# lionl1106/Searchable-Generative-Image-Compression

Measured on AMD Instinct MI355X. Metric: images/sec end-to-end compress (enc+entropy+CLIP) at 256x256, higher is better.
Workload: dtype f32; 1 GPU; configs[1]: batch=32 256x256 encoder+entropy+CLIP compress per GPU, TiTok ViT-L hybrid encoder + ViT-B/32 CLIP, synthetic weights; global_batch=32

## Files before the change

### include/sgic.h

```cpp
#ifndef SGIC_H
#define SGIC_H
#include <stddef.h>
#include <stdint.h>

#ifdef __cplusplus
extern "C" {
#endif

typedef struct ihipStream_t *sgic_stream_t;

#define SGIC_OK 0
#define SGIC_EINVAL -1
#define SGIC_EHIP -2
#define SGIC_ENOSPC -3
#define SGIC_ENODEV -4

const char *sgic_last_error(void);
int sgic_version(void);
int sgic_device_count(void);


int sgic_pmf_to_quantized_cdf(const float *pmf, int n, int precision, uint32_t *cdf_out);

typedef struct sgic_cdf_table sgic_cdf_table;
int sgic_cdf_table_create(const int32_t *cdf, int rows, int cols, const int32_t *sizes, const int32_t *offsets,
                          sgic_cdf_table **out);
void sgic_cdf_table_destroy(sgic_cdf_table *t);

int sgic_rans_encode_batch(const sgic_cdf_table *t, const int16_t *d_sym, const int16_t *d_idx, int B,
                           int n_per_img, uint8_t *d_out, int cap, int32_t *d_off, int32_t *d_len,
                           int32_t *d_err, sgic_stream_t stream);

int sgic_rans_decode_init_batch(const uint8_t *d_streams, int cap, const int32_t *d_off, const int32_t *d_len,
                                int B, uint32_t *d_state, sgic_stream_t stream);
int sgic_rans_decode_batch(const sgic_cdf_table *t, const uint8_t *d_streams, int cap, const int32_t *d_off,
                           const int32_t *d_len, int B, uint32_t *d_state, const int16_t *d_idx, int n,
                           int idx_stride, int16_t *d_sym_out, int out_stride, sgic_stream_t stream);

size_t sgic_pack12_size(size_t n);
int sgic_pack12_batch(const int32_t *d_idx, int B, int n, uint8_t *d_out, sgic_stream_t stream);
int sgic_unpack12_batch(const uint8_t *d_in, int B, int n, int32_t *d_idx, sgic_stream_t stream);

int sgic_quant_step(const float *d_y, const float *d_scales, const float *d_means, int ld_sm, float *d_yhat,
                    int ld_yhat, int B, int H, int W, int C, int k, float thr, int16_t *d_sym, int16_t *d_idx,
                    sgic_stream_t stream);
int sgic_scale_to_index(const float *d_scales, long n, float thr, int16_t *d_idx, sgic_stream_t stream);
int sgic_index_step(const float *d_scales, int ld_sm, int B, int H, int W, int C, int k, float thr,
                    int16_t *d_idx, sgic_stream_t stream);
int sgic_index_margins(const float *d_scales, int ld_sm, int B, int H, int W, int C, int k, float thr, float *d_margin,
                       int16_t *d_alt, sgic_stream_t stream);
int sgic_dequant_step(const int16_t *d_sym, const float *d_means, int ld_sm, float *d_yhat, int ld_yhat, int B,
                      int H, int W, int C, int k, sgic_stream_t stream);

#define SGIC_ACT_NONE 0
#define SGIC_ACT_GELU 1
#define SGIC_ACT_SILU 2
#define SGIC_ACT_TANH 3
#define SGIC_ACT_LRELU 4

typedef struct sgic_profiler sgic_profiler;
typedef struct sgic_launch_opts {
  int tile_mode;
  int attn_mode;
  sgic_profiler *profiler;
  int w_packed;
  int a_packed;
} sgic_launch_opts;

int sgic_profiler_create(sgic_profiler **out);
void sgic_profiler_destroy(sgic_profiler *p);
int sgic_profiler_begin(sgic_profiler *p, int max_launches);
int sgic_profiler_end(sgic_profiler *p, float *ms_out, int cap, int *n_out);

int sgic_gemm_f32(const float *d_A, int lda, const float *d_W, int ldw, const float *d_bias, const float *d_R,
                  int ldr, float *d_C, int ldc, int M, int N, int K, int act, int a_seg, int a_seg_stride,
                  int c_seg, int c_seg_stride, const sgic_launch_opts *opts, sgic_stream_t stream);

int sgic_layernorm_f32(const float *d_x, int ldx, int xseg, int xseg_stride, const float *d_gamma,
                       const float *d_beta, float *d_y, int ldy, int yseg, int yseg_stride, int M, int C, float eps,
                       int act, sgic_stream_t stream);

int sgic_attention_f32(const float *d_q, int ldq, const float *d_k, int ldk, const float *d_v, int ldv,
                       float *d_out, int ldo, int L, int nseq, int nheads, const int32_t *d_rowmap,
                       const float *d_bias, const int32_t *d_biasvar, float scale, const sgic_launch_opts *opts,
                       sgic_stream_t stream);
int sgic_attention_window_f32(const float *d_q, int ldq, const float *d_k, int ldk, const float *d_v, int ldv,
                              float *d_out, int ldo, int L, int nseq, int nheads, const int32_t *d_rowmap,
                              const float *d_bias, const int32_t *d_biasvar, float scale, int q_tok0, int Lq,
                              const sgic_launch_opts *opts, sgic_stream_t stream);
int sgic_copy_blocks_f32(const float *d_src, long src_stride, float *d_dst, long dst_stride, long block_elems, int nblocks,
                         sgic_stream_t stream);

int sgic_im2col_patch(const float *d_x, int B, int C, int H, int W, int P, float mul, float add, int tile16,
                      float *d_out, sgic_stream_t stream);
int sgic_assemble_tokens(const float *d_emb, const float *d_cls, const float *d_pos, const float *d_lat,
                         const float *d_latpos, int N, int P, int T, int D, float *d_out, sgic_stream_t stream);
int sgic_add_rows_bcast(const float *d_in, int ldi, int iseg, const float *d_vec, float *d_out, int ldo, int oseg,
                        int Nn, int Lr, int D, sgic_stream_t stream);
int sgic_dwconv_nhwc(const float *d_x, const float *d_w, const float *d_bias, const float *d_prescale, float *d_y,
                     int B, int H, int W, int C, int k, int tile16, sgic_stream_t stream);
int sgic_im2col_2x2(const float *d_x, int B, int H, int W, int C, int tile16, float *d_out, sgic_stream_t stream);
int sgic_gated_lrelu(const float *d_x, float *d_out, int M, int C2, sgic_stream_t stream);
int sgic_colop(const float *d_x, int ldx, const float *d_v, int ldv, int vrows, float *d_y, int ldy, int M, int C,
               int mode, sgic_stream_t stream);
int sgic_fake2d_transpose(const float *d_in, long in_seq_stride, float *d_out, int N, int T, int D,
                          sgic_stream_t stream);
int sgic_vq_argmin(const float *d_z, int ldz, const float *d_codebook, int ncodes, int dim, int M, int l2norm,
                   int32_t *d_idx, sgic_stream_t stream);
int sgic_clip_preprocess(const float *d_x, long img_stride, long ch_stride, int ldx, int B, int H, int W, int OH,
                         int OW, int S, int top, int left, const int32_t *d_bounds_h, const int32_t *d_kk_h,
                         int ksize_h, const int32_t *d_bounds_v, const int32_t *d_kk_v, int ksize_v,
                         const float *mean3, const float *std3, uint8_t *d_tmp_u8, uint8_t *d_tmp_h, float *d_out,
                         sgic_stream_t stream);
int sgic_l2norm_u8(const float *d_x, int ldx, int M, int D, float *d_unit, uint8_t *d_q, sgic_stream_t stream);

int sgic_split3_f32(const float *d_x, int ld, int rows, int cols, int seg, int seg_stride, uint16_t *d_planes,
                    sgic_stream_t stream);
int sgic_split3_pack_f32(const float *d_x, int ld, int rows, int cols, uint16_t *d_planes, sgic_stream_t stream);
int sgic_gemm_split3_f32(const float *d_A, int lda, int a_seg, int a_seg_stride, uint16_t *d_Aplanes,
                         const uint16_t *d_Wplanes, const float *d_bias, const float *d_R, int ldr, float *d_C, int ldc,
                         uint16_t *d_Cplanes, int M, int N, int K, int act, int c_seg, int c_seg_stride,
                         const sgic_launch_opts *opts, sgic_stream_t stream);
int sgic_conv3x3_split3_f32(const uint16_t *d_in_planes, const uint16_t *d_Wplanes, const float *d_bias, const float *d_R,
                            int ldr, float *d_out, int ldc, int B, int H, int W, int Cin, int Cout, int act,
                            const sgic_launch_opts *opts, sgic_stream_t stream);
int sgic_groupnorm_nhwc_split3(const float *d_x, const float *d_gamma, const float *d_beta, int B, int H, int W, int C,
                               int groups, float eps, int swish, double *d_ws, float *d_stats, uint16_t *d_halo_planes,
                               sgic_stream_t stream);
int sgic_halo_copy_split3(const float *d_in, int B, int H, int W, int C, int upsample2x, int tile16, uint16_t *d_halo_planes,
                          sgic_stream_t stream);
int sgic_attention_split3_f32(const float *d_q, int ldq, const float *d_k, int ldk, const float *d_v, int ldv,
                              uint16_t *d_out_planes, long rows, int L, int nseq, int nheads, const int32_t *d_rowmap,
                              const float *d_bias, const int32_t *d_biasvar, float scale, const sgic_launch_opts *opts,
                              sgic_stream_t stream);
int sgic_attention_window_split3_f32(const float *d_q, int ldq, const float *d_k, int ldk, const float *d_v, int ldv,
                                     uint16_t *d_out_planes, long rows, int L, int nseq, int nheads, const int32_t *d_rowmap,
                                     const float *d_bias, const int32_t *d_biasvar, float scale, int q_tok0, int Lq,
                                     const sgic_launch_opts *opts, sgic_stream_t stream);
int sgic_layernorm_split3_f32(const float *d_x, int ldx, int xseg, int xseg_stride, const float *d_gamma,
                              const float *d_beta, uint16_t *d_planes, int M, int C, float eps, int act,
                              sgic_stream_t stream);

int sgic_gemm_batched_f32(const float *d_A, int lda, long strideA, const float *d_W, int ldw, long strideW,
                          const float *d_bias, const float *d_R, int ldr, long strideR, float *d_C, int ldc,
                          long strideC, int M, int N, int K, int act, int batch, const sgic_launch_opts *opts,
                          sgic_stream_t stream);
int sgic_conv3x3_f32(const float *d_in_halo, const float *d_W, const float *d_bias, const float *d_R, int ldr,
                     float *d_out, int ldc, int B, int H, int W, int Cin, int Cout, int act, const sgic_launch_opts *opts,
                     sgic_stream_t stream);
int sgic_groupnorm_nhwc(const float *d_x, const float *d_gamma, const float *d_beta, int B, int H, int W, int C,
                        int groups, float eps, int swish, int halo_out, double *d_ws, float *d_stats, float *d_y,
                        sgic_stream_t stream);
int sgic_halo_copy(const float *d_in, int B, int H, int W, int C, int upsample2x, int tile16, float *d_out,
                   sgic_stream_t stream);
int sgic_softmax_rows(const float *d_x, float *d_y, long M, int L, float scale, sgic_stream_t stream);
int sgic_pixel_shuffle2_tm16(const float *d_in, int B, int H, int W, int C, float *d_out, sgic_stream_t stream);
int sgic_assemble_dec_tokens(const float *d_emb, const float *d_cls, const float *d_mask, const float *d_pos,
                             const float *d_latpos, int N, int P, int T, int D, float *d_out, sgic_stream_t stream);
int sgic_codebook_gather_norm(const int32_t *d_idx, const float *d_codebook, int M, int dim, int ld, float *d_out,
                              sgic_stream_t stream);
int sgic_nhwc3_to_nchw_clamp(const float *d_in, int ld, int B, int H, int W, float *d_out, sgic_stream_t stream);

int sgic_topk_rows(float *d_scores, int nq, int n, int k, float *d_out_scores, int32_t *d_out_idx, sgic_stream_t stream);

int sgic_search_codes_u8_work_bytes(int nq, int n, int D, int k, int splits, int *splits_used, size_t *bytes);
int sgic_search_codes_u8(const uint8_t *d_q, const float *d_rq, const uint8_t *d_db, const float *d_rdb, int nq, int n, int D, int k,
                         int splits, uint8_t *d_work, size_t work_bytes, float *d_out_scores, int32_t *d_out_idx,
                         sgic_stream_t stream);

int sgic_search_codes_f32q_work_bytes(int nq, int n, int D, int k, int splits, int *splits_used, size_t *bytes);
int sgic_search_codes_f32q(const float *d_q, const uint8_t *d_db, const float *d_rdb, int nq, int n, int D, int k, int splits,
                           uint8_t *d_work, size_t work_bytes, float *d_out_scores, int32_t *d_out_idx, sgic_stream_t stream);

int sgic_search_range_u8(const uint8_t *d_q, const float *d_rq, const uint8_t *d_db, const float *d_rdb, int nq, int n, int D,
                         float threshold, int self_join, int splits, long long capacity, uint64_t *d_count, int32_t *d_out_q,
                         int32_t *d_out_d, float *d_out_score, sgic_stream_t stream);

int sgic_search_range_f32q(const float *d_q, const uint8_t *d_db, const float *d_rdb, int nq, int n, int D, float threshold,
                           int splits, long long capacity, uint64_t *d_count, int32_t *d_out_q, int32_t *d_out_d,
                           float *d_out_score, sgic_stream_t stream);

int sgic_pad_replicate(const float *d_in, float *d_out, int BC, int H, int W, int pl, int pr, int pt, int pb,
                       sgic_stream_t stream);

int sgic_u8hwc_to_f32chw_pad(const uint8_t *d_in, float *d_out, int B, int H, int W, int pl, int pr, int pt, int pb,
                             sgic_stream_t stream);

int sgic_u8canvas_to_f32chw_pad(const uint8_t *d_in, const int32_t *h_hw, float *d_out, int B, int Hc, int Wc, int OH, int OW,
                                sgic_stream_t stream);
int sgic_clip_resize_coeffs(int in_size, int out_size, int ksize, int32_t *d_bounds, int32_t *d_kk, sgic_stream_t stream);
int sgic_clip_preprocess_ragged_workspace(int B, const int32_t *h_geo, int S, size_t *bytes);
int sgic_clip_preprocess_ragged(const float *d_x, long img_stride, long ch_stride, int ldx, int B, const int32_t *h_geo, int S,
                                const float *mean3, const float *std3, uint8_t *d_work, size_t work_bytes, float *d_out,
                                sgic_stream_t stream);
int sgic_clip_preprocess_u8canvas_workspace(int B, const int32_t *h_geo, int S, size_t *bytes);
int sgic_clip_preprocess_u8canvas(const uint8_t *d_canvas, int Hc, int Wc, int B, const int32_t *h_geo, int S, const float *mean3,
                                  const float *std3, uint8_t *d_work, size_t work_bytes, float *d_out, sgic_stream_t stream);

int sgic_jpeg_decode_batch(const int32_t *d_params, const uint8_t *d_scan, const uint8_t *d_tabs, const int32_t *d_segs,
                           const uint16_t *d_quant, int32_t *d_work_params, uint16_t *d_work_quant, int16_t *d_coef,
                           uint8_t *d_planes, uint8_t *d_out, int32_t *d_err, int B, int H, int W, int max_blocks,
                           sgic_stream_t stream);

int sgic_jpeg_decode_scans_batch(const int32_t *d_params, const int32_t *d_descs, const uint8_t *d_scan, const uint8_t *d_tabs,
                                 const int32_t *d_segs, const uint16_t *d_quant, int32_t *d_work_params, uint16_t *d_work_quant,
                                 int16_t *d_coef, uint8_t *d_planes, uint8_t *d_out, int32_t *d_err, int B, int H, int W,
                                 long total_blocks, int max_blocks, const int32_t *h_level_start, int nlevels,
                                 sgic_stream_t stream);

int sgic_embed_tokens(const int32_t *d_ids, const float *d_table, const float *d_pos, float *d_out, int B, int L, int D,
                      int vocab, sgic_stream_t stream);
int sgic_gather_eot_rows(const int32_t *d_ids, const float *d_x, int ldx, float *d_out, int B, int L, int D,
                         sgic_stream_t stream);

#ifdef __cplusplus
}
#endif
#endif
```

### searchable-generative-image-compression_amd/clip.py

```python
import math

import numpy as np
import torch

from . import ops
from ._lib import call
from .config import ClipConfig
from .encoder import RabW, rab_forward, rab_forward_last

_PREC = 22


def _bicubic(x):
    a = -0.5
    x = abs(x)
    if x < 1.0:
        return ((a + 2.0) * x - (a + 3.0)) * x * x + 1
    if x < 2.0:
        return (((x - 5) * x + 8) * x - 4) * a
    return 0.0


def pil_coeffs(in_size, out_size):
    scale = in_size / out_size
    fscale = max(scale, 1.0)
    support = 2.0 * fscale
    ksize = int(math.ceil(support)) * 2 + 1
    bounds = np.zeros((out_size, 2), dtype=np.int32)
    kk = np.zeros((out_size, ksize), dtype=np.int32)
    ss = 1.0 / fscale
    for xx in range(out_size):
        center = (xx + 0.5) * scale
        xmin = int(center - support + 0.5)
        xmin = max(xmin, 0)
        xmax = int(center + support + 0.5)
        xmax = min(xmax, in_size) - xmin
        w = [_bicubic((x + xmin - center + 0.5) * ss) for x in range(xmax)]
        ww = 0.0
        for v in w:
            ww += v
        if ww != 0.0:
            w = [v / ww for v in w]
        for x, v in enumerate(w):
            kk[xx, x] = int(-0.5 + v * (1 << _PREC)) if v < 0 else int(0.5 + v * (1 << _PREC))
        bounds[xx] = (xmin, xmax)
    return bounds, kk, ksize


def resize_geometry(H, W, S):
    if H <= W:
        OH, OW = S, int(S * W / H)
    else:
        OH, OW = int(S * H / W), S
    top = int(round((OH - S) / 2.0))
    left = int(round((OW - S) / 2.0))
    return OH, OW, top, left


class ClipHIP:
    def __init__(self, sd, cfg: ClipConfig, device, p="clip.visual", prune_last=True):
        self.cfg, self.device = cfg, device
        self.prune_last = prune_last
        g = lambda k: sd[f"{p}.{k}"].to(device=device, dtype=torch.float32).contiguous()
        Wd = cfg.width
        self.conv_w = sd[f"{p}.conv1.weight"].reshape(Wd, -1).to(device).contiguous()
        self.cls = g("class_embedding").reshape(1, Wd).contiguous()
        self.pos = g("positional_embedding")
        self.lnpre_w, self.lnpre_b = g("ln_pre.weight"), g("ln_pre.bias")
        self.blocks = [RabW(sd, f"{p}.transformer.resblocks.{i}", device) for i in range(cfg.layers)]
        self.lnpost_w, self.lnpost_b = g("ln_post.weight"), g("ln_post.bias")
        self.projT = sd[f"{p}.proj"].t().to(device).contiguous()
        self.mean = np.asarray(cfg.mean, dtype=np.float32)
        self.std = np.asarray(cfg.std, dtype=np.float32)
        self._coef = {}

    def _coeffs(self, H, W):
        key = (H, W)
        if key not in self._coef:
            S = self.cfg.image_size
            OH, OW, top, left = resize_geometry(H, W, S)
            bh, kh, ksh = pil_coeffs(W, OW)
            bv, kv, ksv = pil_coeffs(H, OH)
            d = lambda a: torch.from_numpy(np.ascontiguousarray(a)).to(self.device)
            self._coef[key] = (OH, OW, top, left, d(bh), d(kh), ksh, d(bv), d(kv), ksv)
        return self._coef[key]

    def preprocess(self, x, H=None, W=None, hw=None):
        if hw is not None:
            return self._preprocess_ragged(x, hw)
        B, _, Hp, Wp = x.shape
        H, W = H or Hp, W or Wp
        S = self.cfg.image_size
        OH, OW, top, left, bh, kh, ksh, bv, kv, ksv = self._coeffs(H, W)
        u8 = torch.empty(B * 3 * H * W, dtype=torch.uint8, device=x.device)
        th = torch.empty(B * 3 * H * OW, dtype=torch.uint8, device=x.device)
        out = torch.empty(B, 3, S, S, dtype=torch.float32, device=x.device)
        import ctypes
        call("sgic_clip_preprocess", ops._p(x), ctypes.c_long(x.stride(0)), ctypes.c_long(x.stride(1)), int(x.stride(2)),
             B, H, W, OH, OW, S, top, left, ops._p(bh), ops._p(kh), ksh, ops._p(bv), ops._p(kv), ksv,
             self.mean.ctypes.data_as(ctypes.c_void_p), self.std.ctypes.data_as(ctypes.c_void_p), ops._p(u8), ops._p(th),
             ops._p(out))
        return out

    def _preprocess_ragged(self, x, hw):
        import ctypes
        B, _, Hp, Wp = x.shape
        hw = np.asarray(hw, dtype=np.int64).reshape(B, 2)
        if (hw <= 0).any() or (hw[:, 0] > Hp).any() or (hw[:, 1] > Wp).any():
            raise ValueError(f"extents {hw.tolist()} outside the {Hp}x{Wp} batch")
        S = self.cfg.image_size
        geo = np.array([(h, w) + resize_geometry(h, w, S) for h, w in hw.tolist()], dtype=np.int32)
        nbytes = ctypes.c_size_t(0)
        call("sgic_clip_preprocess_ragged_workspace", B, geo, S, ctypes.byref(nbytes))
        work = torch.empty(nbytes.value, dtype=torch.uint8, device=x.device)
        out = torch.empty(B, 3, S, S, dtype=torch.float32, device=x.device)
        call("sgic_clip_preprocess_ragged", ops._p(x), ctypes.c_long(x.stride(0)), ctypes.c_long(x.stride(1)), int(x.stride(2)), B, geo, S,
             self.mean, self.std, ops._p(work), ctypes.c_size_t(nbytes.value), ops._p(out))
        return out

    def preprocess_u8(self, canvas, hw):
        if canvas.dim() != 4 or canvas.shape[3] != 3 or canvas.dtype != torch.uint8:
            raise ValueError(f"canvas must be (B, Hc, Wc, 3) uint8, got {tuple(canvas.shape)} {canvas.dtype}")
        B, Hc, Wc, _ = canvas.shape
        hw = np.asarray(hw, dtype=np.int64).reshape(B, 2)
        if (hw <= 0).any() or (hw[:, 0] > Hc).any() or (hw[:, 1] > Wc).any():
            raise ValueError(f"extents {hw.tolist()} outside the {Hc}x{Wc} canvas")
        S = self.cfg.image_size
        geo = np.array([(h, w) + resize_geometry(h, w, S) for h, w in hw.tolist()], dtype=np.int32)
        return ops.clip_preprocess_u8canvas(canvas.contiguous(), geo, S, self.mean, self.std)

    def tower(self, pre):
        cfg = self.cfg
        B = pre.shape[0]
        g = cfg.image_size // cfg.patch
        L = g * g + 1
        A = ops.im2col_patch(pre, cfg.patch, 1.0, 0.0, tile16=False)
        emb = ops.gemm(A, self.conv_w)
        X = ops.assemble_tokens(emb, self.cls, self.pos, None, None, B, g * g, 0, cfg.width)
        ops.layernorm(X, self.lnpre_w, self.lnpre_b, out=X)
        if self.prune_last and L > 32:
            for w in self.blocks[:-1]:
                rab_forward(X, w, L, B, cfg.heads)
            pooled = rab_forward_last(X, self.blocks[-1], L, B, cfg.heads, 0, 32, keep=1)
            ops.layernorm(pooled, self.lnpost_w, self.lnpost_b, out=pooled)
        else:
            for w in self.blocks:
                rab_forward(X, w, L, B, cfg.heads)
            pooled = ops.layernorm(X, self.lnpost_w, self.lnpost_b, M=B, x_seg=(1, L))
        z = ops.gemm(pooled, self.projT)
        return ops.l2norm_u8(z)

    def encode(self, x, H=None, W=None, hw=None):
        return self.tower(self.preprocess(x, H, W, hw))

    def encode_u8(self, canvas, hw):
        return self.tower(self.preprocess_u8(canvas, hw))


class ClipTextHIP:

    def __init__(self, sd, cfg: ClipConfig, device, p="clip"):
        self.cfg, self.device = cfg, device
        g = lambda k: sd[f"{p}.{k}"].to(device=device, dtype=torch.float32).contiguous()
        self.table, self.pos = g("token_embedding.weight"), g("positional_embedding")
        self.blocks = [RabW(sd, f"{p}.transformer.resblocks.{i}", device) for i in range(cfg.t_layers)]
        self.lnf_w, self.lnf_b = g("ln_final.weight"), g("ln_final.bias")
        self.projT = sd[f"{p}.text_projection"].t().to(device=device, dtype=torch.float32).contiguous()
        L = self.L = (cfg.ctx + 3) & ~3
        if L != cfg.ctx:
            self.pos = torch.cat([self.pos, torch.zeros(L - cfg.ctx, cfg.t_width, device=device)]).contiguous()
        self.causal = torch.full((L, L), float("-inf")).triu_(1).reshape(1, L, L).to(device).contiguous()

    def encode_text(self, tokens):
        cfg = self.cfg
        ids = torch.as_tensor(np.asarray(tokens.cpu() if torch.is_tensor(tokens) else tokens)).to(torch.int32)
        if ids.dim() != 2 or ids.shape[1] != cfg.ctx:
            raise ValueError(f"tokens must be (B, {cfg.ctx}), got {tuple(ids.shape)}")
        if self.L != cfg.ctx:
            ids = torch.nn.functional.pad(ids, (0, self.L - cfg.ctx))
        ids = ids.to(self.device).contiguous()
        B, L, D = ids.shape[0], self.L, cfg.t_width
        X = torch.empty(B * L, D, dtype=torch.float32, device=self.device)
        call("sgic_embed_tokens", ops._p(ids), ops._p(self.table), ops._p(self.pos), ops._p(X), B, L, D, cfg.vocab)
        for w in self.blocks:
            rab_forward(X, w, L, B, cfg.t_heads, bias=self.causal)
        pooled = torch.empty(B, D, dtype=torch.float32, device=self.device)
        call("sgic_gather_eot_rows", ops._p(ids), ops._p(X), D, ops._p(pooled), B, L, D)
        ops.layernorm(pooled, self.lnf_w, self.lnf_b, out=pooled)
        z = ops.gemm(pooled, self.projT)
        return ops.l2norm_u8(z)[0]
```

### searchable-generative-image-compression_amd/csrc/gemm_split.hip

```cpp
#include <type_traits>

#include "common.h"
#include "gemm_act.h"
#include "profiler.h"
#include "split3.h"

typedef float f32x16 __attribute__((ext_vector_type(16)));
typedef float f32x4 __attribute__((ext_vector_type(4)));
typedef __bf16 bf16x8 __attribute__((ext_vector_type(8)));
typedef unsigned u32x4 __attribute__((ext_vector_type(4)));

template <bool PACK>
__global__ __launch_bounds__(256) void split3_rows_kernel(const float *__restrict__ x, int ld, int rows, int cols, int seg,
                                                          int seg_stride, unsigned short *__restrict__ planes) {
  const int c8 = cols >> 3;
  const long total = (long)rows * c8, plane = (long)rows * cols;
  for (long i = (long)blockIdx.x * 256 + threadIdx.x; i < total; i += (long)gridDim.x * 256) {
    const int r = (int)(i / c8), c = (int)(i - (long)r * c8) * 8;
    const size_t src = (seg ? (size_t)(r / seg) * seg_stride + (r % seg) : (size_t)r) * ld + c;
    const f32x4 v0 = *reinterpret_cast<const f32x4 *>(x + src), v1 = *reinterpret_cast<const f32x4 *>(x + src + 4);
    unsigned p1[4], p2[4], p3[4];
    s3_split_pair(v0[0], v0[1], p1[0], p2[0], p3[0]);
    s3_split_pair(v0[2], v0[3], p1[1], p2[1], p3[1]);
    s3_split_pair(v1[0], v1[1], p1[2], p2[2], p3[2]);
    s3_split_pair(v1[2], v1[3], p1[3], p2[3], p3[3]);
    const size_t dst = PACK ? ((size_t)(c >> 5) * rows + r) * 32 + (c & 31) : (size_t)r * cols + c;
    *reinterpret_cast<u32x4 *>(planes + dst) = u32x4{p1[0], p1[1], p1[2], p1[3]};
    *reinterpret_cast<u32x4 *>(planes + plane + dst) = u32x4{p2[0], p2[1], p2[2], p2[3]};
    *reinterpret_cast<u32x4 *>(planes + 2 * plane + dst) = u32x4{p3[0], p3[1], p3[2], p3[3]};
  }
}

template <int N, int I = 0, typename F>
__device__ __forceinline__ void s3_for(F &&f) {
  if constexpr (I < N) {
    f(IntC<I>{});
    s3_for<N, I + 1>(f);
  }
}

struct S3Args {
  const unsigned short *A, *W;
  const float *bias, *R;
  float *C;
  int M, N, K, ldr, ldc, act;
  int c_seg, c_seg_stride;
  long a_plane, w_plane;
  unsigned short *Cp;
  long c_plane;
  int vec_epilogue;
  int conv_C, conv_H, conv_W;
  int m_base;
  int w_packed;
  int a_packed, a_rows;
  int c_rows;
};

template <int BM, int BN, int PASSES>
__device__ __forceinline__ void s3_tile_epilogue(const S3Args &g, f32x4 (&acc)[BM][BN], float *ep, int em0, int en0, int wm, int wn, int lane) {
  const int l16 = lane & 15, lq = lane >> 4;
  if (g.vec_epilogue) {
    constexpr int BMP = BM / PASSES, RM = 16 * BMP, CN = 16 * BN, LDW = CN + 4, LPR = CN / 4, RPI = 64 / LPR, NIT = (RM + RPI - 1) / RPI;
    constexpr bool EXACT = (64 % LPR) == 0 && (RM % RPI) == 0;
    static_assert(BM % PASSES == 0, "epilogue passes");
    const int c4 = (lane % LPR) * 4, r0 = lane / LPR;
    const bool lane_on = EXACT || lane < RPI * LPR;
    const int n = en0 + wn + c4;
    const bool colok = n < g.N && lane_on;
    const int nc = colok ? n : 0;
    f32x4 bv = {0.f, 0.f, 0.f, 0.f};
    if (g.bias && colok) bv = *reinterpret_cast<const f32x4 *>(g.bias + n);
    s3_for<PASSES>([&](auto pass_c) __attribute__((always_inline)) {
      constexpr int pass = decltype(pass_c)::value;
#pragma unroll
      for (int i = 0; i < BMP; i++)
#pragma unroll
        for (int j = 0; j < BN; j++) *reinterpret_cast<f32x4 *>(ep + (i * 16 + l16) * LDW + j * 16 + 4 * lq) = acc[pass * BMP + i][j];
      asm volatile("s_waitcnt lgkmcnt(0)" ::: "memory");
      const int wmp = wm + pass * RM;
      auto run = [&](auto act_c, auto res_c, auto pl_c) __attribute__((always_inline)) {
        constexpr int ACT = decltype(act_c)::value;
        constexpr bool HASR = decltype(res_c)::value != 0, PLANES = decltype(pl_c)::value != 0;
        constexpr int EB = NIT < 8 ? NIT : 8;
#pragma unroll
        for (int b = 0; b < NIT; b += EB) {
          f32x4 cv[EB], rv[EB];
#pragma unroll
          for (int q = 0; q < EB; ++q) {
            const int rr = EXACT ? (b + q) * RPI + r0 : min((b + q) * RPI + r0, RM - 1);
            cv[q] = *reinterpret_cast<const f32x4 *>(ep + rr * LDW + c4);
            if constexpr (HASR) rv[q] = *reinterpret_cast<const f32x4 *>(g.R + (size_t)(min(em0 + wmp + rr, g.M - 1) + g.m_base) * g.ldr + nc);
          }
#pragma unroll
          for (int q = 0; q < EB; ++q) {
            if (!EXACT && (b + q >= NIT || (b + q) * RPI + r0 >= RM)) continue;
            const int m = em0 + wmp + (b + q) * RPI + r0;
            f32x4 v = cv[q];
#pragma unroll
            for (int t = 0; t < 4; t++) v[t] = apply_act_c<ACT>(v[t] + bv[t]);
            if constexpr (HASR) v += rv[q];
            if (colok && m < g.M) {
              if constexpr (PLANES) {
                s3_store4(g.Cp, g.c_plane, s3_pack_off(m + g.m_base, n, g.c_rows), v);
              } else {
                const int mm = m + g.m_base;
                const size_t crow = g.c_seg ? (size_t)(mm / g.c_seg) * g.c_seg_stride + (mm % g.c_seg) : (size_t)mm;
                *reinterpret_cast<f32x4 *>(g.C + crow * g.ldc + n) = v;
              }
            }
          }
        }
      };
      auto run_act = [&](auto act_c) __attribute__((always_inline)) {
        if (g.Cp) {
          if (g.R) run(act_c, IntC<1>{}, IntC<1>{});
          else run(act_c, IntC<0>{}, IntC<1>{});
        } else {
          if (g.R) run(act_c, IntC<1>{}, IntC<0>{});
          else run(act_c, IntC<0>{}, IntC<0>{});
        }
      };
      switch (g.act) {
        case ACT_GELU: run_act(IntC<ACT_GELU>{}); break;
        case ACT_SILU: run_act(IntC<ACT_SILU>{}); break;
        case ACT_TANH: run_act(IntC<ACT_TANH>{}); break;
        case ACT_LRELU: run_act(IntC<ACT_LRELU>{}); break;
        default: run_act(IntC<ACT_NONE>{}); break;
      }
    });
    return;
  }
  auto run = [&](auto act_c, auto res_c) __attribute__((always_inline)) {
    constexpr int ACT = decltype(act_c)::value;
    constexpr bool HASR = decltype(res_c)::value != 0;
#pragma unroll
    for (int j = 0; j < BN; j++) {
      const int n = en0 + wn + j * 16 + 4 * lq;
#pragma unroll
      for (int i = 0; i < BM; i++) {
        const int m = em0 + wm + i * 16 + l16;
        if (m >= g.M) continue;
        const int mm = m + g.m_base;
        const size_t crow = g.c_seg ? (size_t)(mm / g.c_seg) * g.c_seg_stride + (mm % g.c_seg) : (size_t)mm;
#pragma unroll
        for (int t = 0; t < 4; t++) {
          if (n + t < g.N) {
            float o = apply_act_c<ACT>(acc[i][j][t] + (g.bias ? g.bias[n + t] : 0.f));
            if constexpr (HASR) o += g.R[(size_t)mm * g.ldr + n + t];
            g.C[crow * g.ldc + n + t] = o;
          }
        }
      }
    }
  };
  auto run_act = [&](auto act_c) __attribute__((always_inline)) {
    if (g.R) run(act_c, IntC<1>{});
    else run(act_c, IntC<0>{});
  };
  switch (g.act) {
    case ACT_GELU: run_act(IntC<ACT_GELU>{}); break;
    case ACT_SILU: run_act(IntC<ACT_SILU>{}); break;
    case ACT_TANH: run_act(IntC<ACT_TANH>{}); break;
    case ACT_LRELU: run_act(IntC<ACT_LRELU>{}); break;
    default: run_act(IntC<ACT_NONE>{}); break;
  }
}

#ifndef S3_ABLATE
#define S3_ABLATE 0
#endif
#ifndef S3_DMA_VARIANT
#define S3_DMA_VARIANT 0
#endif
#ifdef S3_STAMPS
__device__ unsigned long long s3_stamps[4] = {~0ull, 0ull, 0ull, 0ull};
__device__ unsigned long long s3_wg[1024][6];
#endif

template <int WAVES_M, int WAVES_N, int BM, int BN, int NS, int KS, bool PERSIST>
__global__ __launch_bounds__(64 * WAVES_M * WAVES_N, (2 * 3 * 16 * (BM * WAVES_M + BN * WAVES_N) * 64 * KS <= 80 * 1024 && WAVES_M * WAVES_N == 8) ? 2 : 1)
void gemm_split3_kernel(S3Args g) {
#ifdef S3_STAMPS
  const unsigned long long st_rt0 = __builtin_amdgcn_s_memrealtime(), st_c0 = __builtin_amdgcn_s_memtime();
#endif
  static_assert(KS == 1 || KS == 2, "32-k slices per stage");
  static_assert(!PERSIST || NS == 1, "the persistent walk is built on the one-register-set pipeline");
  constexpr int NT = 64 * WAVES_M * WAVES_N, TM = 16 * BM * WAVES_M, TN = 16 * BN * WAVES_N;
  constexpr int ROWB = 64 * KS, SL = 4 * KS;
  constexpr int CA = (TM * SL + NT - 1) / NT, CW = (TN * SL + NT - 1) / NT;
  constexpr int APLANE = TM * ROWB, WPLANE = TN * ROWB, STAGE = 3 * (APLANE + WPLANE);
  constexpr int HB = BN >= 2 ? BN / 2 : BN;
  static_assert((NT / SL) % 16 == 0, "a thread's staged rows must share their swizzle term");
  extern __shared__ __attribute__((aligned(16))) unsigned char smem[];

  const int tiles_m = (g.M + TM - 1) / TM, tiles_n = (g.N + TN - 1) / TN, nwg = tiles_m * tiles_n;
  int m0, n0;
  auto locate = [&](int t) __attribute__((always_inline)) {
    const int q = nwg >> 3, r = nwg & 7, xcd = t & 7, within = t >> 3;
    t = (xcd < r ? xcd * (q + 1) : r * (q + 1) + (xcd - r) * q) + within;
    const int per_group = 8 * tiles_n, group = t / per_group, first_m = group * 8, gsz = min(tiles_m - first_m, 8),
              in_group = t - group * per_group;
    m0 = (first_m + in_group % gsz) * TM;
    n0 = (in_group / gsz) * TN;
  };
  int tile = blockIdx.x;
  locate(tile);
  const int tid = threadIdx.x, lane = tid & 63, wave = tid >> 6;
  const int wm = (wave / WAVES_N) * (16 * BM), wn = (wave % WAVES_N) * (16 * BN);
  auto swz = [](int row) __attribute__((always_inline)) {
    if constexpr (KS == 1) {
      const int gq = (row >> 2) & 3;
      return (((gq ^ (gq >> 1)) & 1) << 1) | (gq >> 1);
    } else {
      return (row >> 1) & 7;
    }
  };
  const int srow = tid / SL, sslot = tid % SL;
  const int sw = srow * ROWB + ((sslot ^ swz(srow)) * 16);
  const unsigned short *aptr[CA], *wptr[CW];
  auto setup = [&]() __attribute__((always_inline)) {
#pragma unroll
    for (int i = 0; i < CA; i++) {
      const int am = min(m0 + srow + i * (NT / SL), g.M - 1);
      if (g.conv_C) {
        const int hw = g.conv_H * g.conv_W, b = am / hw, r = am - b * hw, y = r / g.conv_W, x = r - y * g.conv_W;
        const size_t pix = ((size_t)b * (g.conv_H + 2) + y) * (g.conv_W + 2) + x;
        aptr[i] = g.a_packed ? g.A + ((size_t)(sslot >> 2) * g.a_rows + pix) * 32 + (sslot & 3) * 8 : g.A + pix * g.conv_C + sslot * 8;
      } else if (g.a_packed) {
        aptr[i] = g.A + ((size_t)(sslot >> 2) * g.a_rows + am) * 32 + (sslot & 3) * 8;
      } else {
        aptr[i] = g.A + (size_t)am * g.K + sslot * 8;
      }
    }
#pragma unroll
    for (int i = 0; i < CW; i++) {
      const size_t wr = (size_t)min(n0 + srow + i * (NT / SL), g.N - 1);
      wptr[i] = g.w_packed ? g.W + ((size_t)(sslot >> 2) * g.N + wr) * 32 + (sslot & 3) * 8 : g.W + wr * g.K + sslot * 8;
    }
  };
  setup();
  const bool a_on = CA * NT == TM * SL || srow < TM, w_on = CW * NT == TN * SL || srow < TN;
  u32x4 ra[NS][3][CA], rw[NS][3][CW];
  auto issue = [&](int k0, auto set_c) __attribute__((always_inline)) {
    constexpr int S = decltype(set_c)::value;
    if ((S3_ABLATE & 1) && k0 > 0) return;
    size_t ka = g.a_packed ? (size_t)k0 * g.a_rows : (size_t)k0;
    if (g.conv_C) {
      const int tap = k0 / g.conv_C, c0 = k0 - tap * g.conv_C, ky = tap / 3, kx = tap - 3 * ky;
      ka = g.a_packed ? ((size_t)(c0 >> 5) * g.a_rows + ky * (g.conv_W + 2) + kx) * 32 : (size_t)((ky * (g.conv_W + 2) + kx) * g.conv_C + c0);
    }
    const size_t kw = g.w_packed ? (size_t)k0 * g.N : (size_t)k0;
#pragma unroll
    for (int p = 0; p < 3; p++) {
#pragma unroll
      for (int i = 0; i < CA; i++) ra[S][p][i] = *reinterpret_cast<const u32x4 *>(aptr[i] + p * g.a_plane + ka);
#pragma unroll
      for (int i = 0; i < CW; i++) rw[S][p][i] = *reinterpret_cast<const u32x4 *>(wptr[i] + p * g.w_plane + kw);
    }
  };
  auto store = [&](int buf, auto set_c) __attribute__((always_inline)) {
    constexpr int S = decltype(set_c)::value;
    if ((S3_ABLATE & 2) && buf > 0) return;
    unsigned char *base = smem + buf * STAGE + sw;
#pragma unroll
    for (int p = 0; p < 3; p++) {
      if (a_on) {
#pragma unroll
        for (int i = 0; i < CA; i++) *reinterpret_cast<u32x4 *>(base + p * APLANE + i * (NT / SL) * ROWB) = ra[S][p][i];
      }
      if (w_on) {
#pragma unroll
        for (int i = 0; i < CW; i++) *reinterpret_cast<u32x4 *>(base + 3 * APLANE + p * WPLANE + i * (NT / SL) * ROWB) = rw[S][p][i];
      }
    }
  };
  f32x4 acc[BM][BN];
  const int l16 = lane & 15, lq = lane >> 4;
  int foff[KS];
#pragma unroll
  for (int ks = 0; ks < KS; ks++) foff[ks] = l16 * ROWB + (((4 * ks + lq) ^ swz(l16)) * 16);
  const int abase = wm * ROWB, bbase = 3 * APLANE + wn * ROWB;
  bf16x8 wf[3][BN], af[2][3];
  bool frag_reads = true;
  auto read_w = [&](int buf, int j, int ks) __attribute__((always_inline)) {
    if ((S3_ABLATE & 8) && !frag_reads) return;
    const unsigned char *base = smem + buf * STAGE + bbase + j * 16 * ROWB + foff[ks];
#pragma unroll
    for (int p = 0; p < 3; p++) wf[p][j] = *reinterpret_cast<const bf16x8 *>(base + p * WPLANE);
  };
  auto read_a = [&](int buf, int i, int set, int ks) __attribute__((always_inline)) {
    if ((S3_ABLATE & 8) && !frag_reads) return;
    const unsigned char *base = smem + buf * STAGE + abase + i * 16 * ROWB + foff[ks];
#pragma unroll
    for (int p = 0; p < 3; p++) af[set][p] = *reinterpret_cast<const bf16x8 *>(base + p * APLANE);
  };
  auto block = [&](int i, int j, int set) __attribute__((always_inline)) {
    f32x4 c = acc[i][j];
    c = __builtin_amdgcn_mfma_f32_16x16x32_bf16(wf[0][j], af[set][2], c, 0, 0, 0);
    c = __builtin_amdgcn_mfma_f32_16x16x32_bf16(wf[2][j], af[set][0], c, 0, 0, 0);
    c = __builtin_amdgcn_mfma_f32_16x16x32_bf16(wf[1][j], af[set][1], c, 0, 0, 0);
    c = __builtin_amdgcn_mfma_f32_16x16x32_bf16(wf[0][j], af[set][1], c, 0, 0, 0);
    c = __builtin_amdgcn_mfma_f32_16x16x32_bf16(wf[1][j], af[set][0], c, 0, 0, 0);
    c = __builtin_amdgcn_mfma_f32_16x16x32_bf16(wf[0][j], af[set][0], c, 0, 0, 0);
    acc[i][j] = c;
  };
  constexpr int BKS = 32 * KS;
  const int nk = g.K / BKS;
  auto tile_prologue = [&]() __attribute__((always_inline)) {
#pragma unroll
    for (int i = 0; i < BM; i++)
#pragma unroll
      for (int j = 0; j < BN; j++) acc[i][j] = f32x4{0.f, 0.f, 0.f, 0.f};
    store(0, IntC<0>{});
    if constexpr (NS == 1) {
      if (nk > 1) issue(BKS, IntC<0>{});
    } else {
      s3_for<NS>([&](auto u_c) __attribute__((always_inline)) {
        constexpr int J = decltype(u_c)::value + 1;
        if (J < nk) issue(J * BKS, IntC<J % NS>{});
      });
    }
    asm volatile("s_waitcnt lgkmcnt(0)" ::: "memory");
    __builtin_amdgcn_s_barrier();
#pragma unroll
    for (int j = BN - HB; j < BN; j++) read_w(0, j, 0);
    read_a(0, 0, 0, 0);
    if (S3_ABLATE & 8) {
#pragma unroll
      for (int j = 0; j < BN; j++) read_w(0, j, 0);
      read_a(0, 0, 1, 0);
      frag_reads = false;
    }
  };
  issue(0, IntC<0>{});
  auto compute = [&](int cur, auto ks_c, bool more) __attribute__((always_inline)) {
    constexpr int KSI = decltype(ks_c)::value;
    constexpr bool LAST = KSI == KS - 1;
    const int nxt = cur ^ 1;
    if constexpr (BN >= 2) {
#pragma unroll
      for (int j = 0; j < BN - HB; j++) read_w(cur, j, KSI);
    }
#pragma unroll
    for (int i = 0; i < BM; i++) {
      const int set = i & 1;
      if (i + 1 < BM) read_a(cur, i + 1, set ^ 1, KSI);
#pragma unroll
      for (int j = BN - HB; j < BN; j++) block(i, j, set);
      if (i == BM - 1) {
        if constexpr (LAST) {
          if constexpr (NS == 1) {
            constexpr int NMF1 = 6 * (BM * BN - (BN - HB)), NDW = 3 * (CA + CW), NDR1 = 3 * (BN - HB) + 3 * (BM - 1);
#pragma unroll
            for (int q = 0; q < NMF1; q++) {
              __builtin_amdgcn_sched_group_barrier(0x008, 1, 0);
              if (q < NDW) __builtin_amdgcn_sched_group_barrier(0x200, 1, 0);
              else if (q < 2 * NDW) __builtin_amdgcn_sched_group_barrier(0x020, 1, 0);
              if (q % 4 == 0 && q / 4 < NDR1) __builtin_amdgcn_sched_group_barrier(0x100, 1, 0);
            }
          }
          asm volatile("s_waitcnt lgkmcnt(0)" ::: "memory");
          if (!(S3_ABLATE & 4)) __builtin_amdgcn_s_barrier();
          if (more) {
#pragma unroll
            for (int j = BN - HB; j < BN; j++) read_w(nxt, j, 0);
            read_a(nxt, 0, BM == 1 ? 0 : (BM & 1), 0);
          }
        } else {
#pragma unroll
          for (int j = BN - HB; j < BN; j++) read_w(cur, j, KSI + 1);
          read_a(cur, 0, BM == 1 ? 0 : (BM & 1), KSI + 1);
        }
      }
      if constexpr (BN >= 2) {
#pragma unroll
        for (int j = 0; j < BN - HB; j++) block(i, j, set);
      }
    }
  };
  static_assert((BM == 1 && BN == 1) || (BM % 2) == 0, "A row 0 of the next slice must land in set 0, free at that point");
  auto tile_mainloop = [&]() __attribute__((always_inline)) {
    auto stage_mfma = [&](int cur, bool more) __attribute__((always_inline)) {
      s3_for<KS>([&](auto ks_c) __attribute__((always_inline)) { compute(cur, ks_c, more); });
    };
    if constexpr (NS == 1) {
      auto stage = [&](int kt, auto store_c, auto issue_c) __attribute__((always_inline)) {
        constexpr bool ST = decltype(store_c)::value, IS = decltype(issue_c)::value;
        if constexpr (ST) store((kt & 1) ^ 1, IntC<0>{});
        if constexpr (IS) issue((kt + 2) * BKS, IntC<0>{});
        stage_mfma(kt & 1, ST);
      };
      using T = std::true_type;
      using F = std::false_type;
      int kt = 0;
      for (; kt + 2 < nk; ++kt) stage(kt, T{}, T{});
      if (kt + 1 < nk) {
        stage(kt, T{}, F{});
        ++kt;
      }
      stage(kt, F{}, F{});
    } else {
      for (int base = 0; base < nk; base += NS) {
        s3_for<NS>([&](auto u_c) __attribute__((always_inline)) {
          constexpr int U = decltype(u_c)::value;
          const int kt = base + U;
          if (kt < nk) {
            const bool more = kt + 1 < nk;
            if (more) {
              store((kt & 1) ^ 1, IntC<(U + 1) % NS>{});
              if (kt + 1 + NS < nk) issue((kt + 1 + NS) * BKS, IntC<(U + 1) % NS>{});
            }
            stage_mfma(kt & 1, more);
          }
        });
      }
    }
  };

  auto tile_epilogue = [&](int em0, int en0) __attribute__((always_inline)) {
    s3_tile_epilogue<BM, BN, 1>(g, acc, reinterpret_cast<float *>(smem) + wave * (16 * BM * (16 * BN + 4)), em0, en0, wm, wn, lane);
  };

#ifdef S3_STAMPS
  unsigned long long ph_pro = 0, ph_main = 0, ph_epi = 0, ph_tiles = 0;
#endif
  for (;;) {
#ifdef S3_STAMPS
    const unsigned long long ph0 = __builtin_amdgcn_s_memtime();
#endif
    tile_prologue();
#ifdef S3_STAMPS
    const unsigned long long ph1 = __builtin_amdgcn_s_memtime();
// ... 262 lines not shown
    if (!more_tiles) break;
  }
}

template <int WAVES_M, int WAVES_N, int BM, int BN, int KS, int RING>
__global__ __launch_bounds__(64 * WAVES_M * WAVES_N, 1)
void gemm_split3_ring_kernel(S3Args g) {
  constexpr int NW = WAVES_M * WAVES_N, TM = 16 * BM * WAVES_M, TN = 16 * BN * WAVES_N;
  constexpr int ROWB = 64, PA = TM / 16, PW = TN / 16, PP = PA + PW, NP = 3 * PP * KS;
  constexpr int C = (NP + NW - 1) / NW;
  constexpr int APLANE = TM * ROWB, WPLANE = TN * ROWB, SLICE = 3 * (APLANE + WPLANE), STEP = KS * SLICE;
  static_assert(RING >= 3 && (RING - 2) * C <= 63, "vmcnt is a 6-bit counter");
  static_assert(NW * 16 * BM * (16 * BN + 4) * 4 <= RING * STEP, "the epilogue's per-wave slices fit the ring");
  extern __shared__ __attribute__((aligned(16))) unsigned char smem[];

  const int tiles_m = (g.M + TM - 1) / TM, tiles_n = (g.N + TN - 1) / TN, nwg = tiles_m * tiles_n;
  int m0, n0;
  {
    int t = blockIdx.x;
    const int q = nwg >> 3, r = nwg & 7, xcd = t & 7, within = t >> 3;
    t = (xcd < r ? xcd * (q + 1) : r * (q + 1) + (xcd - r) * q) + within;
    const int per_group = 8 * tiles_n, group = t / per_group, first_m = group * 8, gsz = min(tiles_m - first_m, 8),
              in_group = t - group * per_group;
    m0 = (first_m + in_group % gsz) * TM;
    n0 = (in_group / gsz) * TN;
  }
  const int tid = threadIdx.x, lane = tid & 63, wave = __builtin_amdgcn_readfirstlane(tid >> 6);
  const int wm = (wave / WAVES_N) * (16 * BM), wn = (wave % WAVES_N) * (16 * BN);
  auto swz = [](int row) __attribute__((always_inline)) {
    const int gq = (row >> 2) & 3;
    return (((gq ^ (gq >> 1)) & 1) << 1) | (gq >> 1);
  };
  const int prow = lane >> 2, pslot = (lane & 3) ^ swz(prow);
  const char *src[C];
  size_t kmul[C];
  unsigned dst[C];
#pragma unroll
  for (int i = 0; i < C; i++) {
    const int f = (wave + NW * i) % NP, ks = f / (3 * PP), rem = f - ks * (3 * PP), p = rem / PP, r = rem - p * PP;
    const bool isA = r < PA;
    const int rw = isA ? min(m0 + r * 16 + prow, g.M - 1) : min(n0 + (r - PA) * 16 + prow, g.N - 1);
    const unsigned short *base = isA ? g.A + p * g.a_plane : g.W + p * g.w_plane;
    const bool packed = isA ? g.a_packed != 0 : g.w_packed != 0;
    const size_t prows = isA ? (size_t)g.a_rows : (size_t)g.N;
    src[i] = reinterpret_cast<const char *>(base + (packed ? ((size_t)ks * prows + rw) * 32 : (size_t)rw * g.K + ks * 32)) + pslot * 16;
    kmul[i] = packed ? prows * (64 * KS) : (size_t)(64 * KS);
    dst[i] = (unsigned)(ks * SLICE + (isA ? p * APLANE + r * 1024 : 3 * APLANE + p * WPLANE + (r - PA) * 1024));
  }
  auto dma = [&](int step, int slot) __attribute__((always_inline)) {
    unsigned char *sbase = smem + slot * STEP;
#pragma unroll
    for (int i = 0; i < C; i++)
      __builtin_amdgcn_global_load_lds((s3_glb_void *)(src[i] + (size_t)step * kmul[i]), (s3_lds_void *)(sbase + dst[i]), 16, 0, 0);
  };
  f32x4 acc[BM][BN];
#pragma unroll
  for (int i = 0; i < BM; i++)
#pragma unroll
    for (int j = 0; j < BN; j++) acc[i][j] = f32x4{0.f, 0.f, 0.f, 0.f};
  const int l16 = lane & 15, lq = lane >> 4;
  const int foff = l16 * ROWB + ((lq ^ swz(l16)) * 16);
  const int abase = wm * ROWB + foff, bbase = 3 * APLANE + wn * ROWB + foff;
  bf16x8 af[2][KS][BM][3], wf[2][KS][BN][3];
  auto read_frags = [&](int slot, auto set_c) __attribute__((always_inline)) {
    constexpr int S = decltype(set_c)::value;
    const unsigned char *sbase = smem + slot * STEP;
#pragma unroll
    for (int ks = 0; ks < KS; ks++) {
#pragma unroll
      for (int p = 0; p < 3; p++) {
#pragma unroll
        for (int i = 0; i < BM; i++) af[S][ks][i][p] = *reinterpret_cast<const bf16x8 *>(sbase + ks * SLICE + p * APLANE + i * 16 * ROWB + abase);
#pragma unroll
        for (int j = 0; j < BN; j++) wf[S][ks][j][p] = *reinterpret_cast<const bf16x8 *>(sbase + ks * SLICE + p * WPLANE + j * 16 * ROWB + bbase);
      }
    }
  };
  auto compute = [&](auto set_c) __attribute__((always_inline)) {
    constexpr int S = decltype(set_c)::value;
    constexpr int TW[6] = {0, 2, 1, 0, 1, 0}, TA[6] = {2, 0, 1, 1, 0, 0};
#pragma unroll
    for (int ks = 0; ks < KS; ks++)
#pragma unroll
      for (int t = 0; t < 6; t++)
#pragma unroll
        for (int i = 0; i < BM; i++)
#pragma unroll
          for (int j = 0; j < BN; j++)
            acc[i][j] = __builtin_amdgcn_mfma_f32_16x16x32_bf16(wf[S][ks][j][TW[t]], af[S][ks][i][TA[t]], acc[i][j], 0, 0, 0);
  };
  const int nsteps = g.K / (32 * KS);
  {
    const int npro = min(RING - 1, nsteps);
    for (int s = 0; s < npro; s++) dma(s, s);
    if (npro == RING - 1) asm volatile("s_waitcnt vmcnt(%0)" ::"n"((RING - 2) * C) : "memory");
    else asm volatile("s_waitcnt vmcnt(0)" ::: "memory");
    __builtin_amdgcn_s_barrier();
    read_frags(0, IntC<0>{});
  }
  int slot_next = 1 % RING;
  int slot_fill = (RING - 1) % RING;
  auto iter = [&](int s, auto set_c) __attribute__((always_inline)) {
    constexpr int S = decltype(set_c)::value;
    if (s + 1 < nsteps) {
      if (s + RING - 2 <= nsteps - 1) asm volatile("s_waitcnt vmcnt(%0) lgkmcnt(0)" ::"n"((RING - 3) * C) : "memory");
      else asm volatile("s_waitcnt vmcnt(0) lgkmcnt(0)" ::: "memory");
      __builtin_amdgcn_s_barrier();
      if (s + RING - 1 < nsteps) dma(s + RING - 1, slot_fill);
      read_frags(slot_next, IntC<S ^ 1>{});
      slot_next = slot_next + 1 == RING ? 0 : slot_next + 1;
      slot_fill = slot_fill + 1 == RING ? 0 : slot_fill + 1;
    }
    compute(set_c);
  };
  for (int s = 0; s < nsteps; s += 2) {
    iter(s, IntC<0>{});
    if (s + 1 < nsteps) iter(s + 1, IntC<1>{});
  }
  asm volatile("s_waitcnt vmcnt(0) lgkmcnt(0)" ::: "memory");
  __builtin_amdgcn_s_barrier();
  s3_tile_epilogue<BM, BN, 1>(g, acc, reinterpret_cast<float *>(smem) + wave * (16 * BM * (16 * BN + 4)), m0, n0, wm, wn, lane);
}

extern "C" int sgic_split3_f32(const float *d_x, int ld, int rows, int cols, int seg, int seg_stride, uint16_t *d_planes,
                               sgic_stream_t stream) {
  SGIC_REQUIRE(d_x && d_planes && rows > 0 && cols > 0, "null/empty");
  SGIC_REQUIRE((cols & 7) == 0 && (ld & 3) == 0 && ld >= cols, "cols % 8, ld % 4");
  SGIC_REQUIRE(((uintptr_t)d_x & 15) == 0 && ((uintptr_t)d_planes & 15) == 0, "16-byte alignment");
  SGIC_REQUIRE(seg >= 0 && (seg == 0 || seg_stride >= seg), "row segment map");
  const long total = (long)rows * (cols >> 3);
  const unsigned grid = (unsigned)min((total + 255) / 256, 256L * 16);
  split3_rows_kernel<false><<<grid, 256, 0, to_stream(stream)>>>(d_x, ld, rows, cols, seg, seg_stride, d_planes);
  return sgic::check_launch("split3_rows_kernel");
}

extern "C" int sgic_split3_pack_f32(const float *d_x, int ld, int rows, int cols, uint16_t *d_planes, sgic_stream_t stream) {
  SGIC_REQUIRE(d_x && d_planes && rows > 0 && cols > 0, "null/empty");
  SGIC_REQUIRE((cols & 31) == 0 && (ld & 3) == 0 && ld >= cols, "cols % 32, ld % 4");
  SGIC_REQUIRE(((uintptr_t)d_x & 15) == 0 && ((uintptr_t)d_planes & 15) == 0, "16-byte alignment");
  const long total = (long)rows * (cols >> 3);
  const unsigned grid = (unsigned)min((total + 255) / 256, 256L * 16);
  split3_rows_kernel<true><<<grid, 256, 0, to_stream(stream)>>>(d_x, ld, rows, cols, 0, 0, d_planes);
  return sgic::check_launch("split3_rows_kernel<pack>");
}

#define SGIC_SPLIT3_TILE_MODES 31

template <int WAVES_M, int WAVES_N, int BM, int BN, int NS, int KS = 1, bool PERSIST = false>
static int s3_launch(const S3Args &g, hipStream_t st, hipEvent_t ev_start, hipEvent_t ev_stop) {
  constexpr int NT = 64 * WAVES_M * WAVES_N, TM = 16 * BM * WAVES_M, TN = 16 * BN * WAVES_N;
  constexpr int LDS = 2 * 3 * (TM + TN) * 64 * KS;
  static bool attr_set[64] = {};
  auto kernel = gemm_split3_kernel<WAVES_M, WAVES_N, BM, BN, NS, KS, PERSIST>;
  int dev = 0;
  SGIC_HIP(hipGetDevice(&dev));
  if (dev < 0 || dev >= 64 || !attr_set[dev]) {
    SGIC_HIP(hipFuncSetAttribute(reinterpret_cast<const void *>(kernel), hipFuncAttributeMaxDynamicSharedMemorySize, LDS));
    if (dev >= 0 && dev < 64) attr_set[dev] = true;
  }
  unsigned ntiles = (unsigned)(((g.M + TM - 1) / TM) * ((g.N + TN - 1) / TN));
  const dim3 grid(PERSIST ? (ntiles < 256u ? ntiles : 256u) : ntiles);
  if (ev_start || ev_stop) {
    hipExtLaunchKernelGGL(kernel, grid, dim3(NT), LDS, st, ev_start, ev_stop, 0, g);
  } else {
    kernel<<<grid, NT, LDS, st>>>(g);
  }
  return sgic::check_launch("gemm_split3_kernel");
}

template <int WAVES_M, int WAVES_N, int BM, int BN, bool PERSIST = false, bool WS1 = false>
static int s3_launch_dma(const S3Args &g, hipStream_t st, hipEvent_t ev_start, hipEvent_t ev_stop) {
  constexpr int NT = 64 * WAVES_M * WAVES_N, TM = 16 * BM * WAVES_M, TN = 16 * BN * WAVES_N;
  constexpr int LDS = WS1 ? 3 * (2 * TM + TN) * 64 : 2 * 3 * (TM + TN) * 64;
  static_assert(LDS <= 160 * 1024, "LDS of a CU");
  static bool attr_set[64] = {};
  auto kernel = gemm_split3_dma_kernel<WAVES_M, WAVES_N, BM, BN, PERSIST, WS1>;
  int dev = 0;
  SGIC_HIP(hipGetDevice(&dev));
  if (dev < 0 || dev >= 64 || !attr_set[dev]) {
    SGIC_HIP(hipFuncSetAttribute(reinterpret_cast<const void *>(kernel), hipFuncAttributeMaxDynamicSharedMemorySize, LDS));
    if (dev >= 0 && dev < 64) attr_set[dev] = true;
  }
  unsigned ntiles = (unsigned)(((g.M + TM - 1) / TM) * ((g.N + TN - 1) / TN));
  const dim3 grid(PERSIST ? (ntiles < 256u ? ntiles : 256u) : ntiles);
  if (ev_start || ev_stop) {
    hipExtLaunchKernelGGL(kernel, grid, dim3(NT), LDS, st, ev_start, ev_stop, 0, g);
  } else {
    kernel<<<grid, NT, LDS, st>>>(g);
  }
  return sgic::check_launch("gemm_split3_dma_kernel");
}

template <int WAVES_M, int WAVES_N, int BM, int BN, int KS, int RING>
static int s3_launch_ring(const S3Args &g, hipStream_t st, hipEvent_t ev_start, hipEvent_t ev_stop) {
  constexpr int NT = 64 * WAVES_M * WAVES_N, TM = 16 * BM * WAVES_M, TN = 16 * BN * WAVES_N;
  constexpr int LDS = RING * KS * 3 * (TM + TN) * 64;
  static_assert(LDS <= 160 * 1024, "LDS of a CU");
  static bool attr_set[64] = {};
  auto kernel = gemm_split3_ring_kernel<WAVES_M, WAVES_N, BM, BN, KS, RING>;
  int dev = 0;
  SGIC_HIP(hipGetDevice(&dev));
  if (dev < 0 || dev >= 64 || !attr_set[dev]) {
    SGIC_HIP(hipFuncSetAttribute(reinterpret_cast<const void *>(kernel), hipFuncAttributeMaxDynamicSharedMemorySize, LDS));
    if (dev >= 0 && dev < 64) attr_set[dev] = true;
  }
  const dim3 grid((unsigned)(((g.M + TM - 1) / TM) * ((g.N + TN - 1) / TN)));
  if (ev_start || ev_stop) {
    hipExtLaunchKernelGGL(kernel, grid, dim3(NT), LDS, st, ev_start, ev_stop, 0, g);
  } else {
    kernel<<<grid, NT, LDS, st>>>(g);
  }
  return sgic::check_launch("gemm_split3_ring_kernel");
}

static int s3_mode(const S3Args &g, int mode, hipStream_t st, hipEvent_t e0, hipEvent_t e1) {
  const bool dma_ok = (size_t)(g.a_packed ? 32 : g.K) * 2 * 256 < (1ull << 31) && (size_t)(g.w_packed ? 32 : g.K) * 2 * 256 < (1ull << 31) &&
                      (!g.conv_C || (size_t)(g.conv_W + 2) * (g.a_packed ? 32 : g.conv_C) * 2 * 1024 < (1ull << 31));
  switch (mode) {
    case 1: return dma_ok ? s3_launch_dma<2, 4, 4, 4>(g, st, e0, e1) : s3_launch<2, 4, 2, 2, 1>(g, st, e0, e1);
    case 10: return dma_ok ? s3_launch_dma<2, 4, 4, 4, true>(g, st, e0, e1) : s3_launch<2, 4, 2, 2, 1>(g, st, e0, e1);
#ifndef S3_MICRO_BIG_ONLY
    case 14: return dma_ok ? s3_launch_dma<4, 2, 4, 4>(g, st, e0, e1) : s3_launch<2, 4, 2, 2, 1>(g, st, e0, e1);
    case 15: return dma_ok ? s3_launch_dma<4, 2, 4, 4, true>(g, st, e0, e1) : s3_launch<2, 4, 2, 2, 1>(g, st, e0, e1);
    case 28: return dma_ok ? s3_launch_dma<2, 4, 4, 3>(g, st, e0, e1) : s3_launch<2, 4, 4, 2, 1>(g, st, e0, e1);
    case 29: return dma_ok ? s3_launch_dma<2, 4, 4, 3, true>(g, st, e0, e1) : s3_launch<2, 4, 4, 2, 1>(g, st, e0, e1);
    case 30: return dma_ok ? s3_launch_dma<2, 4, 8, 4, false, true>(g, st, e0, e1) : s3_launch<2, 4, 2, 2, 1>(g, st, e0, e1);
    case 16: return dma_ok ? s3_launch_dma<2, 4, 4, 2>(g, st, e0, e1) : s3_launch<2, 4, 4, 2, 1>(g, st, e0, e1);
    case 17: return dma_ok ? s3_launch_dma<2, 4, 4, 2, true>(g, st, e0, e1) : s3_launch<2, 4, 4, 2, 1, 1, true>(g, st, e0, e1);
    case 2: return s3_launch<2, 4, 4, 2, 1>(g, st, e0, e1);
    case 18: return (!g.conv_C && g.K % 64 == 0) ? s3_launch_ring<2, 2, 1, 1, 2, 6>(g, st, e0, e1) : s3_mode(g, 4, st, e0, e1);
    case 19: return (!g.conv_C && g.K % 64 == 0) ? s3_launch_ring<2, 2, 2, 1, 2, 4>(g, st, e0, e1) : s3_mode(g, 4, st, e0, e1);
    case 20: return (!g.conv_C && g.K % 64 == 0) ? s3_launch_ring<2, 2, 1, 2, 2, 4>(g, st, e0, e1) : s3_mode(g, 4, st, e0, e1);
    case 21: return !g.conv_C ? s3_launch_ring<2, 2, 2, 2, 1, 6>(g, st, e0, e1) : s3_mode(g, 3, st, e0, e1);
    case 22: return !g.conv_C ? s3_launch_ring<2, 4, 2, 1, 1, 6>(g, st, e0, e1) : s3_mode(g, 3, st, e0, e1);
    case 23: return !g.conv_C ? s3_launch_ring<1, 4, 5, 1, 1, 5>(g, st, e0, e1) : s3_mode(g, 3, st, e0, e1);
    case 24: return !g.conv_C ? s3_launch_ring<1, 3, 5, 1, 1, 6>(g, st, e0, e1) : s3_mode(g, 3, st, e0, e1);
    case 25: return (!g.conv_C && g.K % 64 == 0) ? s3_launch_ring<2, 3, 1, 1, 2, 5>(g, st, e0, e1) : s3_mode(g, 4, st, e0, e1);
    case 11: return s3_launch<2, 4, 4, 2, 1, 1, true>(g, st, e0, e1);
    case 3: return s3_launch<2, 2, 2, 2, 4>(g, st, e0, e1);
    case 4: return (g.K % 64 == 0 && g.conv_C % 64 == 0) ? s3_launch<2, 2, 1, 1, 3, 2>(g, st, e0, e1) : s3_launch<2, 2, 1, 1, 6>(g, st, e0, e1);
    default: return s3_launch<2, 4, 2, 2, 1>(g, st, e0, e1);
#else
    default: return SGIC_EINVAL;
#endif
  }
}

static int s3_dispatch(const S3Args &g, const sgic_launch_opts *opts, hipStream_t st) {
  const int M = g.M, N = g.N, K = g.K;
  int mode = opts ? opts->tile_mode : 0;
  SGIC_REQUIRE(mode >= 0 && mode <= SGIC_SPLIT3_TILE_MODES, "tile_mode");
  if (!mode) {
    const long t256 = (long)((M + 127) / 128) * ((N + 255) / 256), t128 = (long)((M + 127) / 128) * ((N + 127) / 128),
               t64 = (long)((M + 63) / 64) * ((N + 63) / 64);
    mode = t256 >= 512 ? 1 : (t128 >= 384 ? 2 : (t64 >= 256 ? 3 : 4));
  }
  const auto *evp = prof_next(opts);
  hipEvent_t e0 = evp ? evp->first : nullptr, e1 = evp ? evp->second : nullptr;
  if (mode == 31) {
    const long tiles_n = (N + 255) / 256, tiles_m = (M + 255) / 256;
    const long m_full = (tiles_m * tiles_n / 256) * 256 / tiles_n, m_split = m_full * 256;
    if (m_full > 0 && m_split < M && !g.conv_C) {
      S3Args g1 = g, g2 = g;
      g1.M = (int)m_split;
      g2.M = M - (int)m_split;
      g2.A += g.a_packed ? m_split * 32 : m_split * K;
      g2.m_base = (int)m_split;
      int rc = s3_mode(g1, 30, st, e0, nullptr);
      if (rc) return rc;
      return s3_mode(g2, 1, st, nullptr, e1);
    }
    mode = 30;
  }
  if ((mode >= 6 && mode <= 9) || mode == 12 || mode == 13 || mode == 26 || mode == 27) {
    const bool ring_tail = mode >= 26;
    const int cm = ring_tail ? (mode == 26 ? 8 : 12) : mode;
    const int big = cm >= 12 ? cm - 11 : (cm >= 8 ? cm - 7 : cm - 5), tail = ring_tail ? 23 : (cm >= 8 ? 4 : 5), TM = 128, TN = big == 1 ? 256 : 128;
    const int big_mode = cm >= 12 ? big + 9 : big;
    const long tiles_n = (N + TN - 1) / TN, tiles_m = (M + TM - 1) / TM;
    const long m_full = (tiles_m * tiles_n / 256) * 256 / tiles_n;
    const long m_split = m_full * TM;
    if (m_full > 0 && m_split < M && !g.conv_C) {
      S3Args g1 = g, g2 = g;
      g1.M = (int)m_split;
      g2.M = M - (int)m_split;
      g2.A += g.a_packed ? m_split * 32 : m_split * K;
      g2.m_base = (int)m_split;
      int rc = s3_mode(g1, big_mode, st, e0, nullptr);
      if (rc) return rc;
      return s3_mode(g2, tail, st, nullptr, e1);
    }
    mode = big_mode;
  }
  return s3_mode(g, mode, st, e0, e1);
}

extern "C" int sgic_gemm_split3_f32(const float *d_A, int lda, int a_seg, int a_seg_stride, uint16_t *d_Aplanes,
                                    const uint16_t *d_Wplanes, const float *d_bias, const float *d_R, int ldr, float *d_C,
                                    int ldc, uint16_t *d_Cplanes, int M, int N, int K, int act, int c_seg, int c_seg_stride,
                                    const sgic_launch_opts *opts, sgic_stream_t stream) {
  SGIC_REQUIRE(d_Aplanes && d_Wplanes && (d_C || d_Cplanes) && M > 0 && N > 0 && K > 0, "null/empty");
  SGIC_REQUIRE((K & 31) == 0, "K must be a multiple of 32");
  SGIC_REQUIRE(((uintptr_t)d_Aplanes & 15) == 0 && ((uintptr_t)d_Wplanes & 15) == 0, "planes must be 16-byte aligned");
  SGIC_REQUIRE((d_Cplanes || ldc >= N) && (!d_R || ldr >= N), "leading dimensions");
  SGIC_REQUIRE(act >= 0 && act <= ACT_LRELU, "activation");
  SGIC_REQUIRE(c_seg >= 0 && (c_seg == 0 || c_seg_stride >= c_seg), "row segment map");
  int a_packed = opts ? opts->a_packed : 0;
  if (d_A) {
    SGIC_REQUIRE((lda & 3) == 0 && lda >= K && ((uintptr_t)d_A & 15) == 0 && a_seg >= 0 && (a_seg == 0 || a_seg_stride >= a_seg), "A operand");
    const long total = (long)M * (K >> 3);
    split3_rows_kernel<true><<<(unsigned)min((total + 255) / 256, 256L * 16), 256, 0, to_stream(stream)>>>(d_A, lda, M, K, a_seg, a_seg_stride, d_Aplanes);
    int rc = sgic::check_launch("split3_rows_kernel<pack>");
    if (rc) return rc;
    a_packed = 1;
  }
  SGIC_REQUIRE(!d_Cplanes || (N & 31) == 0, "planes output needs N % 32 == 0");
  const int vec = (N % 4 == 0) && (!d_bias || ((uintptr_t)d_bias & 15) == 0) && (!d_R || ((ldr % 4 == 0) && ((uintptr_t)d_R & 15) == 0)) &&
                  (d_Cplanes ? ((uintptr_t)d_Cplanes & 7) == 0 : ((ldc % 4 == 0) && ((uintptr_t)d_C & 15) == 0));
  SGIC_REQUIRE(!d_Cplanes || (vec && c_seg == 0), "planes output needs float4-addressable operands and no row map");
  S3Args g{d_Aplanes, d_Wplanes, d_bias, d_R, d_C, M, N, K, ldr, ldc, act, c_seg, c_seg_stride, (long)M * K, (long)N * K, d_Cplanes, (long)M * N, vec, 0, 0, 0, 0,
           opts ? opts->w_packed : 0, a_packed, M, M};
  return s3_dispatch(g, opts, to_stream(stream));
}

extern "C" int sgic_conv3x3_split3_f32(const uint16_t *d_in_planes, const uint16_t *d_Wplanes, const float *d_bias,
                                       const float *d_R, int ldr, float *d_out, int ldc, int B, int H, int W, int Cin, int Cout,
                                       int act, const sgic_launch_opts *opts, sgic_stream_t stream) {
  const long Ml = (long)B * H * W, halo_rows = (long)B * (H + 2) * (W + 2);
  SGIC_REQUIRE(d_in_planes && d_Wplanes && d_out && B > 0 && H > 0 && W > 0 && Cout > 0, "null/empty");
  SGIC_REQUIRE(Ml < (1l << 31), "too many pixels");
  SGIC_REQUIRE(Cin > 0 && Cin % 32 == 0, "implicit-GEMM conv needs Cin % 32 == 0");
  SGIC_REQUIRE(((uintptr_t)d_in_planes & 15) == 0 && ((uintptr_t)d_Wplanes & 15) == 0, "planes must be 16-byte aligned");
  SGIC_REQUIRE(ldc >= Cout && (!d_R || ldr >= Cout) && act >= 0 && act <= ACT_LRELU, "leading dimensions / activation");
  const int M = (int)Ml, N = Cout, K = 9 * Cin;
  const int vec = (N % 4 == 0) && (!d_bias || ((uintptr_t)d_bias & 15) == 0) && (!d_R || ((ldr % 4 == 0) && ((uintptr_t)d_R & 15) == 0)) &&
                  (ldc % 4 == 0) && ((uintptr_t)d_out & 15) == 0;
  S3Args g{d_in_planes, d_Wplanes, d_bias, d_R, d_out, M, N, K, ldr, ldc, act, 0, 0, halo_rows * Cin, (long)N * K, nullptr, 0, vec, Cin, H, W, 0,
           opts ? opts->w_packed : 0, opts ? opts->a_packed : 0, (int)halo_rows, 0};
  return s3_dispatch(g, opts, to_stream(stream));
}
```

### searchable-generative-image-compression_amd/csrc/misc.hip

```cpp
#include "common.h"
#include <limits.h>

typedef float f32x4 __attribute__((ext_vector_type(4)));

__device__ __forceinline__ long fmap_row(int b, int y, int x, int H, int W, int tile16) {
  if (!tile16) return ((long)b * H + y) * W + x;
  const int nH = H >> 4, nW = W >> 4;
  return ((((long)b * nH + (y >> 4)) * nW + (x >> 4)) << 8) + ((y & 15) << 4) + (x & 15);
}

#define GRID_STRIDE(i, n) for (long i = (long)blockIdx.x * blockDim.x + threadIdx.x; i < (n); i += (long)gridDim.x * blockDim.x)
static inline unsigned ew_grid(long n) {
  long g = (n + 255) / 256;
  return (unsigned)(g < 1 ? 1 : (g > 8192 ? 8192 : g));
}

__global__ void im2col_patch_kernel(const float *__restrict__ x, int B, int C, int H, int W, int P, float mul, float add,
                                    int tile16, float *__restrict__ out) {
  const int gh = H / P, gw = W / P, K = C * P * P, P4 = P >> 2;
  const long total = (long)B * gh * gw * C * P * P4;
  GRID_STRIDE(i, total) {
    long t = i;
    const int kx4 = (int)(t % P4);
    t /= P4;
    const int ky = (int)(t % P);
    t /= P;
    const int c = (int)(t % C);
    t /= C;
    const int gx = (int)(t % gw);
    t /= gw;
    const int gy = (int)(t % gh);
    const int b = (int)(t / gh);
    f32x4 v = *reinterpret_cast<const f32x4 *>(x + (((long)b * C + c) * H + gy * P + ky) * W + gx * P + kx4 * 4);
#pragma unroll
    for (int e = 0; e < 4; e++) v[e] = v[e] * mul + add;
    const long row = fmap_row(b, gy, gx, gh, gw, tile16);
    *reinterpret_cast<f32x4 *>(out + row * K + (c * P + ky) * P + kx4 * 4) = v;
  }
}

extern "C" int sgic_im2col_patch(const float *d_x, int B, int C, int H, int W, int P, float mul, float add, int tile16,
                                 float *d_out, sgic_stream_t stream) {
  SGIC_REQUIRE(d_x && d_out && B > 0 && C > 0 && P >= 4 && (P & 3) == 0 && H % P == 0 && W % P == 0, "args");
  SGIC_REQUIRE(!tile16 || ((H / P) % 16 == 0 && (W / P) % 16 == 0), "tile-major order needs a patch grid multiple of 16");
  SGIC_REQUIRE((W & 3) == 0 && ((uintptr_t)d_x & 15) == 0 && ((uintptr_t)d_out & 15) == 0, "alignment");
  const long total = (long)B * (H / P) * (W / P) * C * P * (P / 4);
  im2col_patch_kernel<<<ew_grid(total), 256, 0, to_stream(stream)>>>(d_x, B, C, H, W, P, mul, add, tile16, d_out);
  return sgic::check_launch("im2col_patch_kernel");
}

__global__ void assemble_tokens_kernel(const float *__restrict__ emb, const float *__restrict__ cls,
                                       const float *__restrict__ pos, const float *__restrict__ lat,
                                       const float *__restrict__ latpos, int N, int P, int T, int D,
                                       float *__restrict__ out) {
  const int L = 1 + P + T, D4 = D >> 2;
  const long total = (long)N * L * D4;
  GRID_STRIDE(i, total) {
    const int d4 = (int)(i % D4);
    const long r = i / D4;
    const int l = (int)(r % L);
    const int n = (int)(r / L);
    f32x4 a, b;
    if (l == 0) {
      a = reinterpret_cast<const f32x4 *>(cls)[d4];
      b = reinterpret_cast<const f32x4 *>(pos)[d4];
    } else if (l <= P) {
      a = reinterpret_cast<const f32x4 *>(emb + ((long)n * P + (l - 1)) * D)[d4];
      b = reinterpret_cast<const f32x4 *>(pos + (long)l * D)[d4];
    } else {
      a = reinterpret_cast<const f32x4 *>(lat + (long)(l - 1 - P) * D)[d4];
      b = reinterpret_cast<const f32x4 *>(latpos + (long)(l - 1 - P) * D)[d4];
    }
    reinterpret_cast<f32x4 *>(out + r * D)[d4] = a + b;
  }
}

extern "C" int sgic_assemble_tokens(const float *d_emb, const float *d_cls, const float *d_pos, const float *d_lat,
                                    const float *d_latpos, int N, int P, int T, int D, float *d_out,
                                    sgic_stream_t stream) {
  SGIC_REQUIRE(d_emb && d_cls && d_pos && d_out && N > 0 && P > 0 && T >= 0 && D > 0 && (D & 3) == 0, "args");
  SGIC_REQUIRE(T == 0 || (d_lat && d_latpos), "latent tokens");
  const long total = (long)N * (1 + P + T) * (D / 4);
  assemble_tokens_kernel<<<ew_grid(total), 256, 0, to_stream(stream)>>>(d_emb, d_cls, d_pos, d_lat, d_latpos, N, P, T, D,
                                                                         d_out);
  return sgic::check_launch("assemble_tokens_kernel");
}

__global__ void add_rows_bcast_kernel(const float *__restrict__ in, int ldi, int iseg, const float *__restrict__ vec,
                                      float *__restrict__ out, int ldo, int oseg, int Nn, int Lr, int D) {
  const int D4 = D >> 2;
  const long total = (long)Nn * Lr * D4;
  GRID_STRIDE(i, total) {
    const int d4 = (int)(i % D4);
    const long r = i / D4;
    const int l = (int)(r % Lr);
    const int n = (int)(r / Lr);
    f32x4 a = reinterpret_cast<const f32x4 *>(in + ((long)n * iseg + l) * ldi)[d4];
    if (vec) a += reinterpret_cast<const f32x4 *>(vec + (long)l * D)[d4];
    reinterpret_cast<f32x4 *>(out + ((long)n * oseg + l) * ldo)[d4] = a;
  }
}

extern "C" int sgic_add_rows_bcast(const float *d_in, int ldi, int iseg, const float *d_vec, float *d_out, int ldo,
                                   int oseg, int Nn, int Lr, int D, sgic_stream_t stream) {
  SGIC_REQUIRE(d_in && d_out && Nn > 0 && Lr > 0 && D > 0 && (D & 3) == 0 && (ldi & 3) == 0 && (ldo & 3) == 0, "args");
  const long total = (long)Nn * Lr * (D / 4);
  add_rows_bcast_kernel<<<ew_grid(total), 256, 0, to_stream(stream)>>>(d_in, ldi, iseg, d_vec, d_out, ldo, oseg, Nn, Lr, D);
  return sgic::check_launch("add_rows_bcast_kernel");
}

__global__ void dwconv_kernel(const float *__restrict__ x, const float *__restrict__ w, const float *__restrict__ bias,
                              const float *__restrict__ prescale, float *__restrict__ y, int B, int H, int W, int C,
                              int k, int tile16) {
  const int C4 = C >> 2, pad = k >> 1;
  const long total = (long)B * H * W * C4;
  GRID_STRIDE(i, total) {
    const int c4 = (int)(i % C4);
    long t = i / C4;
    const int xx = (int)(t % W);
    t /= W;
    const int yy = (int)(t % H);
    const int b = (int)(t / H);
    f32x4 acc = bias ? reinterpret_cast<const f32x4 *>(bias)[c4] : f32x4{0.f, 0.f, 0.f, 0.f};
    f32x4 ps = prescale ? reinterpret_cast<const f32x4 *>(prescale)[c4] : f32x4{1.f, 1.f, 1.f, 1.f};
    for (int ky = 0; ky < k; ky++) {
      const int sy = yy + ky - pad;
      if (sy < 0 || sy >= H) continue;
      for (int kx = 0; kx < k; kx++) {
        const int sx = xx + kx - pad;
        if (sx < 0 || sx >= W) continue;
        f32x4 v = reinterpret_cast<const f32x4 *>(x + fmap_row(b, sy, sx, H, W, tile16) * C)[c4];
        if (prescale) v *= ps;
        const f32x4 wv = reinterpret_cast<const f32x4 *>(w + (long)(ky * k + kx) * C)[c4];
        acc += v * wv;
      }
    }
    reinterpret_cast<f32x4 *>(y + fmap_row(b, yy, xx, H, W, tile16) * C)[c4] = acc;
  }
}

template <int KS>
__global__ __launch_bounds__(256) void dwconv_x4_kernel(const float *__restrict__ x, const float *__restrict__ w,
                                                        const float *__restrict__ bias, const float *__restrict__ prescale,
                                                        float *__restrict__ y, int B, int H, int W, int C, int tile16) {
  constexpr int pad = KS >> 1;
  const int C4 = C >> 2, XG = W >> 2;
  const long total = (long)B * H * XG * C4;
  long blk = blockIdx.x;
  if ((gridDim.x & 7) == 0) blk = (long)(blockIdx.x & 7) * (gridDim.x >> 3) + (blockIdx.x >> 3);
  for (long i = blk * 256 + threadIdx.x; i < total; i += (long)gridDim.x * 256) {
    const int c4 = (int)(i % C4);
    long t = i / C4;
    const int x0 = (int)(t % XG) * 4;
    t /= XG;
    const int yy = (int)(t % H);
    const int b = (int)(t / H);
    const f32x4 bz = bias ? reinterpret_cast<const f32x4 *>(bias)[c4] : f32x4{0.f, 0.f, 0.f, 0.f};
    const f32x4 ps = prescale ? reinterpret_cast<const f32x4 *>(prescale)[c4] : f32x4{1.f, 1.f, 1.f, 1.f};
    f32x4 acc[4] = {bz, bz, bz, bz};
#pragma unroll
    for (int ky = 0; ky < KS; ky++) {
      const int sy = yy + ky - pad;
      if (sy < 0 || sy >= H) continue;
      f32x4 in[KS + 3];
#pragma unroll
      for (int j = 0; j < KS + 3; j++) {
        const int sx = x0 + j - pad;
        f32x4 v = {0.f, 0.f, 0.f, 0.f};
        if (sx >= 0 && sx < W) {
          v = reinterpret_cast<const f32x4 *>(x + fmap_row(b, sy, sx, H, W, tile16) * C)[c4];
          if (prescale) v *= ps;
        }
        in[j] = v;
      }
#pragma unroll
      for (int kx = 0; kx < KS; kx++) {
        const f32x4 wv = reinterpret_cast<const f32x4 *>(w + (long)(ky * KS + kx) * C)[c4];
#pragma unroll
        for (int o = 0; o < 4; o++) acc[o] += in[o + kx] * wv;
      }
    }
#pragma unroll
    for (int o = 0; o < 4; o++) reinterpret_cast<f32x4 *>(y + fmap_row(b, yy, x0 + o, H, W, tile16) * C)[c4] = acc[o];
  }
}

extern "C" int sgic_dwconv_nhwc(const float *d_x, const float *d_w, const float *d_bias, const float *d_prescale,
                                float *d_y, int B, int H, int W, int C, int k, int tile16, sgic_stream_t stream) {
  SGIC_REQUIRE(d_x && d_w && d_y && d_x != d_y && B > 0 && H > 0 && W > 0 && C > 0 && (C & 3) == 0 && (k & 1) == 1, "args");
  SGIC_REQUIRE(!tile16 || (H % 16 == 0 && W % 16 == 0), "tile-major layout needs H,W multiples of 16");
  const long total = (long)B * H * W * (C / 4);
  if ((W & 3) == 0 && (k == 3 || k == 5)) {
    const unsigned grid = (unsigned)((total / 4 + 255) / 256);
    if (k == 5) dwconv_x4_kernel<5><<<grid, 256, 0, to_stream(stream)>>>(d_x, d_w, d_bias, d_prescale, d_y, B, H, W, C, tile16);
    else dwconv_x4_kernel<3><<<grid, 256, 0, to_stream(stream)>>>(d_x, d_w, d_bias, d_prescale, d_y, B, H, W, C, tile16);
    return sgic::check_launch("dwconv_x4_kernel");
  }
  dwconv_kernel<<<ew_grid(total), 256, 0, to_stream(stream)>>>(d_x, d_w, d_bias, d_prescale, d_y, B, H, W, C, k, tile16);
  return sgic::check_launch("dwconv_kernel");
}

__global__ void im2col_2x2_kernel(const float *__restrict__ x, int B, int H, int W, int C, int tile16,
                                  float *__restrict__ out) {
  const int C4 = C >> 2, OH = H >> 1, OW = W >> 1;
  const long total = (long)B * OH * OW * 4 * C4;
  GRID_STRIDE(i, total) {
    const int c4 = (int)(i % C4);
    long t = i / C4;
    const int kk = (int)(t & 3);
    t >>= 2;
    const int ox = (int)(t % OW);
    t /= OW;
    const int oy = (int)(t % OH);
    const int b = (int)(t / OH);
    const f32x4 v = reinterpret_cast<const f32x4 *>(x + fmap_row(b, oy * 2 + (kk >> 1), ox * 2 + (kk & 1), H, W, tile16) * C)[c4];
    reinterpret_cast<f32x4 *>(out + ((((long)b * OH + oy) * OW + ox) * 4 + kk) * C)[c4] = v;
  }
}

extern "C" int sgic_im2col_2x2(const float *d_x, int B, int H, int W, int C, int tile16, float *d_out,
                               sgic_stream_t stream) {
  SGIC_REQUIRE(d_x && d_out && B > 0 && H > 0 && W > 0 && (H & 1) == 0 && (W & 1) == 0 && (C & 3) == 0, "args");
  const long total = (long)B * (H / 2) * (W / 2) * C;
  im2col_2x2_kernel<<<ew_grid(total), 256, 0, to_stream(stream)>>>(d_x, B, H, W, C, tile16, d_out);
  return sgic::check_launch("im2col_2x2_kernel");
}

__global__ void gated_lrelu_kernel(const float *__restrict__ x, float *__restrict__ out, long M, int C2) {
  const int C4 = C2 >> 2;
  const long total = M * C4;
  GRID_STRIDE(i, total) {
    const int c4 = (int)(i % C4);
    const long m = i / C4;
    const f32x4 a = reinterpret_cast<const f32x4 *>(x + m * 2 * C2)[c4];
    const f32x4 b = reinterpret_cast<const f32x4 *>(x + m * 2 * C2 + C2)[c4];
    f32x4 o;
#pragma unroll
    for (int e = 0; e < 4; e++) o[e] = (a[e] >= 0.f ? a[e] : 0.1f * a[e]) + (b[e] >= 0.f ? b[e] : 0.01f * b[e]);
    reinterpret_cast<f32x4 *>(out + m * C2)[c4] = o;
  }
}

extern "C" int sgic_gated_lrelu(const float *d_x, float *d_out, int M, int C2, sgic_stream_t stream) {
  SGIC_REQUIRE(d_x && d_out && M > 0 && C2 > 0 && (C2 & 3) == 0, "args");
  gated_lrelu_kernel<<<ew_grid((long)M * C2 / 4), 256, 0, to_stream(stream)>>>(d_x, d_out, M, C2);
  return sgic::check_launch("gated_lrelu_kernel");
}

__global__ void colop_kernel(const float *__restrict__ x, int ldx, const float *__restrict__ v, int ldv, int vrows,
                             float *__restrict__ y, int ldy, long M, int C, int mode) {
  const int C4 = C >> 2;
  const long total = M * C4;
  GRID_STRIDE(i, total) {
    const int c4 = (int)(i % C4);
    const long m = i / C4;
    const f32x4 a = reinterpret_cast<const f32x4 *>(x + m * ldx)[c4];
    const f32x4 b = reinterpret_cast<const f32x4 *>(v + (m % vrows) * ldv)[c4];
    f32x4 o;
#pragma unroll
    for (int e = 0; e < 4; e++) o[e] = mode == 0 ? a[e] * b[e] : (mode == 1 ? a[e] / fmaxf(b[e], 0.5f) : a[e] * fmaxf(b[e], 0.5f));
    reinterpret_cast<f32x4 *>(y + m * ldy)[c4] = o;
  }
}

extern "C" int sgic_colop(const float *d_x, int ldx, const float *d_v, int ldv, int vrows, float *d_y, int ldy, int M,
                          int C, int mode, sgic_stream_t stream) {
  SGIC_REQUIRE(d_x && d_v && d_y && M > 0 && C > 0 && (C & 3) == 0 && vrows > 0 && (mode >= 0 && mode <= 2), "args");
  SGIC_REQUIRE((ldx & 3) == 0 && (ldv & 3) == 0 && (ldy & 3) == 0, "leading dims multiple of 4");
  colop_kernel<<<ew_grid((long)M * C / 4), 256, 0, to_stream(stream)>>>(d_x, ldx, d_v, ldv, vrows, d_y, ldy, M, C, mode);
  return sgic::check_launch("colop_kernel");
}

__global__ void fake2d_transpose_kernel(const float *__restrict__ in, long in_seq_stride, float *__restrict__ out, int N,
                                        int T, int D) {
  const long total = (long)N * T * D;
  GRID_STRIDE(i, total) {
    const int c = (int)(i % D);
    const long r = i / D;
    const int t = (int)(r % T);
    const int n = (int)(r / T);
    out[i] = in[(long)n * in_seq_stride + (long)c * T + t];
  }
}

extern "C" int sgic_fake2d_transpose(const float *d_in, long in_seq_stride, float *d_out, int N, int T, int D,
                                     sgic_stream_t stream) {
  SGIC_REQUIRE(d_in && d_out && N > 0 && T > 0 && D > 0, "args");
  fake2d_transpose_kernel<<<ew_grid((long)N * T * D), 256, 0, to_stream(stream)>>>(d_in, in_seq_stride, d_out, N, T, D);
  return sgic::check_launch("fake2d_transpose_kernel");
}

extern "C" int sgic_copy_blocks_f32(const float *d_src, long src_stride, float *d_dst, long dst_stride, long block_elems,
                                    int nblocks, sgic_stream_t stream) {
  SGIC_REQUIRE(d_src && d_dst && block_elems > 0 && nblocks > 0, "args");
  SGIC_REQUIRE(src_stride >= block_elems && dst_stride >= block_elems, "strides");
  SGIC_HIP(hipMemcpy2DAsync(d_dst, (size_t)dst_stride * 4, d_src, (size_t)src_stride * 4, (size_t)block_elems * 4, (size_t)nblocks,
                            hipMemcpyDeviceToDevice, to_stream(stream)));
  return SGIC_OK;
}

#define VQ_TPW 4
__global__ __launch_bounds__(256) void vq_argmin_kernel(const float *__restrict__ z, int ldz, const float *__restrict__ cb,
                                                        int ncodes, int dim, int M, int l2norm, int *__restrict__ idx) {
  __shared__ float s_z[VQ_TPW][17];
  __shared__ float s_best[4][VQ_TPW];
  __shared__ int s_besti[4][VQ_TPW];
  const int tid = threadIdx.x, lane = tid & 63, wave = tid >> 6;
  const int m0 = blockIdx.x * VQ_TPW;
  if (tid < VQ_TPW) {
    const int m = min(m0 + tid, M - 1);
    float zv[16];
    float zn = 0.f;
#pragma unroll
    for (int d = 0; d < 16; d++) {
      zv[d] = d < dim ? z[(long)m * ldz + d] : 0.f;
      if (d < dim) zn += zv[d] * zv[d];
    }
    if (l2norm) {
      const float inv = 1.0f / fmaxf(sqrtf(zn), 1e-12f);
      zn = 0.f;
#pragma unroll
      for (int d = 0; d < 16; d++) {
        zv[d] *= inv;
        if (d < dim) zn += zv[d] * zv[d];
      }
    }
#pragma unroll
    for (int d = 0; d < 16; d++) s_z[tid][d] = zv[d];
    s_z[tid][16] = zn;
  }
  __syncthreads();
  float best[VQ_TPW];
  int besti[VQ_TPW];
#pragma unroll
  for (int t = 0; t < VQ_TPW; t++) best[t] = INFINITY, besti[t] = 0x7fffffff;
  for (int c = tid; c < ncodes; c += 256) {
    float ev[16];
    float en = 0.f;
#pragma unroll
    for (int d = 0; d < 16; d++) {
      ev[d] = d < dim ? cb[(long)c * dim + d] : 0.f;
      if (d < dim) en += ev[d] * ev[d];
    }
    if (l2norm) {
      const float inv = 1.0f / fmaxf(sqrtf(en), 1e-12f);
      en = 0.f;
#pragma unroll
      for (int d = 0; d < 16; d++) {
        ev[d] *= inv;
        if (d < dim) en += ev[d] * ev[d];
      }
    }
#pragma unroll
    for (int t = 0; t < VQ_TPW; t++) {
      float dot = 0.f;
#pragma unroll
      for (int d = 0; d < 16; d++)
        if (d < dim) dot += s_z[t][d] * ev[d];
      const float dist = s_z[t][16] + en - 2.0f * dot;
      if (dist < best[t]) best[t] = dist, besti[t] = c;
    }
  }
#pragma unroll
  for (int t = 0; t < VQ_TPW; t++) {
    float b = best[t];
    int bi = besti[t];
#pragma unroll
    for (int o = 32; o > 0; o >>= 1) {
      const float ob = __shfl_xor(b, o);
      const int oi = __shfl_xor(bi, o);
      if (ob < b || (ob == b && oi < bi)) b = ob, bi = oi;
    }
    if (lane == 0) s_best[wave][t] = b, s_besti[wave][t] = bi;
  }
  __syncthreads();
  if (tid < VQ_TPW && m0 + tid < M) {
    float b = s_best[0][tid];
    int bi = s_besti[0][tid];
    for (int w = 1; w < 4; w++) {
      const float ob = s_best[w][tid];
      const int oi = s_besti[w][tid];
      if (ob < b || (ob == b && oi < bi)) b = ob, bi = oi;
    }
    idx[m0 + tid] = bi;
  }
}

extern "C" int sgic_vq_argmin(const float *d_z, int ldz, const float *d_codebook, int ncodes, int dim, int M, int l2norm,
                              int32_t *d_idx, sgic_stream_t stream) {
  SGIC_REQUIRE(d_z && d_codebook && d_idx && M > 0 && ncodes > 0 && dim > 0 && dim <= 16 && ldz >= dim, "args");
  vq_argmin_kernel<<<cdiv(M, VQ_TPW), 256, 0, to_stream(stream)>>>(d_z, ldz, d_codebook, ncodes, dim, M, l2norm, d_idx);
  return sgic::check_launch("vq_argmin_kernel");
}

__global__ void to_u8_kernel(const float *__restrict__ x, long img_stride, long ch_stride, int ldx, int B, int H, int W,
                             uint8_t *__restrict__ out) {
  const long total = (long)B * 3 * H * W;
  GRID_STRIDE(i, total) {
    const int xx = (int)(i % W);
    long t = i / W;
    const int yy = (int)(t % H);
    t /= H;
    const int c = (int)(t % 3);
    const int b = (int)(t / 3);
    float v = x[b * img_stride + c * ch_stride + (long)yy * ldx + xx];
    v = fminf(fmaxf(v, -1.f), 1.f);
    v = (v * 0.5f + 0.5f) * 255.f;
    out[i] = (uint8_t)v;
  }
}

__global__ void resize_h_kernel(const uint8_t *__restrict__ in, int B3, int H, int W, int OW, const int *__restrict__ bounds,
                                const int *__restrict__ kk, int ksize, uint8_t *__restrict__ out) {
  const long total = (long)B3 * H * OW;
  GRID_STRIDE(i, total) {
    const int xx = (int)(i % OW);
    const long row = i / OW;
    const int xmin = bounds[2 * xx], cnt = bounds[2 * xx + 1];
    int ss = 1 << 21;
    const uint8_t *p = in + row * W + xmin;
    const int *k = kk + xx * ksize;
    for (int x = 0; x < cnt; x++) ss += (int)p[x] * k[x];
    ss >>= 22;
    out[i] = (uint8_t)(ss < 0 ? 0 : (ss > 255 ? 255 : ss));
  }
}

__global__ void resize_v_crop_norm_kernel(const uint8_t *__restrict__ in, int B, int H, int OW, int S, int top, int left,
                                          const int *__restrict__ bounds, const int *__restrict__ kk, int ksize,
                                          float m0, float m1, float m2, float s0, float s1, float s2,
                                          float *__restrict__ out) {
  const long total = (long)B * 3 * S * S;
  GRID_STRIDE(i, total) {
    const int xx = (int)(i % S);
    long t = i / S;
    const int yy = (int)(t % S);
    t /= S;
    const int c = (int)(t % 3);
    const int b = (int)(t / 3);
    const int oy = yy + top, ox = xx + left;
    const int ymin = bounds[2 * oy], cnt = bounds[2 * oy + 1];
    const int *k = kk + oy * ksize;
    const uint8_t *p = in + ((long)(b * 3 + c) * H + ymin) * OW + ox;
    int ss = 1 << 21;
    for (int y = 0; y < cnt; y++) ss += (int)p[(long)y * OW] * k[y];
    ss >>= 22;
    const int u = ss < 0 ? 0 : (ss > 255 ? 255 : ss);
    const float mean = c == 0 ? m0 : (c == 1 ? m1 : m2), sd = c == 0 ? s0 : (c == 1 ? s1 : s2);
    out[i] = ((float)u / 255.0f - mean) / sd;
  }
}

extern "C" int sgic_clip_preprocess(const float *d_x, long img_stride, long ch_stride, int ldx, int B, int H, int W,
                                    int OH, int OW, int S, int top, int left, const int32_t *d_bounds_h,
                                    const int32_t *d_kk_h, int ksize_h, const int32_t *d_bounds_v, const int32_t *d_kk_v,
                                    int ksize_v, const float *mean3, const float *std3, uint8_t *d_tmp_u8,
                                    uint8_t *d_tmp_h, float *d_out, sgic_stream_t stream) {
  SGIC_REQUIRE(d_x && d_tmp_u8 && d_tmp_h && d_out && mean3 && std3 && B > 0 && H > 0 && W > 0 && S > 0, "args");
  SGIC_REQUIRE(top >= 0 && left >= 0 && top + S <= OH && left + S <= OW, "crop window");
  SGIC_REQUIRE(d_bounds_h && d_kk_h && d_bounds_v && d_kk_v, "coefficient tables");
  hipStream_t st = to_stream(stream);
  to_u8_kernel<<<ew_grid((long)B * 3 * H * W), 256, 0, st>>>(d_x, img_stride, ch_stride, ldx, B, H, W, d_tmp_u8);
  resize_h_kernel<<<ew_grid((long)B * 3 * H * OW), 256, 0, st>>>(d_tmp_u8, B * 3, H, W, OW, d_bounds_h, d_kk_h, ksize_h,
                                                                d_tmp_h);
  resize_v_crop_norm_kernel<<<ew_grid((long)B * 3 * S * S), 256, 0, st>>>(d_tmp_h, B, H, OW, S, top, left, d_bounds_v,
                                                                          d_kk_v, ksize_v, mean3[0], mean3[1], mean3[2],
                                                                          std3[0], std3[1], std3[2], d_out);
  return sgic::check_launch("clip_preprocess");
}

__global__ __launch_bounds__(256) void l2norm_u8_kernel(const float *__restrict__ x, int ldx, int M, int D,
                                                        float *__restrict__ unit, uint8_t *__restrict__ q) {
  const int lane = threadIdx.x & 63;
  const int m = blockIdx.x * 4 + (threadIdx.x >> 6);
  if (m >= M) return;
  float s = 0.f;
  for (int d = lane; d < D; d += 64) {
    const float v = x[(long)m * ldx + d];
    s += v * v;
  }
#pragma unroll
  for (int o = 32; o > 0; o >>= 1) s += __shfl_xor(s, o);
  const float nrm = sqrtf(s);
  for (int d = lane; d < D; d += 64) {
    const float u = x[(long)m * ldx + d] / nrm;
    unit[(long)m * D + d] = u;
    const float r = rintf((u * 0.5f + 0.5f) * 255.0f);
    q[(long)m * D + d] = (uint8_t)fminf(fmaxf(r, 0.f), 255.f);
  }
}

extern "C" int sgic_l2norm_u8(const float *d_x, int ldx, int M, int D, float *d_unit, uint8_t *d_q, sgic_stream_t stream) {
  SGIC_REQUIRE(d_x && d_unit && d_q && M > 0 && D > 0 && ldx >= D, "args");
  l2norm_u8_kernel<<<cdiv(M, 4), 256, 0, to_stream(stream)>>>(d_x, ldx, M, D, d_unit, d_q);
  return sgic::check_launch("l2norm_u8_kernel");
}

__global__ void embed_tokens_kernel(const int *__restrict__ ids, const float *__restrict__ table,
                                    const float *__restrict__ pos, float *__restrict__ out, int B, int L, int D, int vocab) {
  const int D4 = D >> 2;
  const long total = (long)B * L * D4;
  GRID_STRIDE(i, total) {
    const int d4 = (int)(i % D4);
    const long r = i / D4;
    const int l = (int)(r % L);
    int id = ids[r];
    id = id < 0 ? 0 : (id >= vocab ? vocab - 1 : id);
    const f32x4 a = reinterpret_cast<const f32x4 *>(table + (long)id * D)[d4];
    const f32x4 p = reinterpret_cast<const f32x4 *>(pos + (long)l * D)[d4];
    reinterpret_cast<f32x4 *>(out + r * D)[d4] = a + p;
  }
}

extern "C" int sgic_embed_tokens(const int *d_ids, const float *d_table, const float *d_pos, float *d_out, int B, int L,
                                 int D, int vocab, sgic_stream_t stream) {
  SGIC_REQUIRE(d_ids && d_table && d_pos && d_out && B > 0 && L > 0 && D > 0 && (D & 3) == 0 && vocab > 0, "args");
  const long total = (long)B * L * (D / 4);
  embed_tokens_kernel<<<ew_grid(total), 256, 0, to_stream(stream)>>>(d_ids, d_table, d_pos, d_out, B, L, D, vocab);
  return sgic::check_launch("embed_tokens_kernel");
}

__global__ __launch_bounds__(64) void gather_eot_rows_kernel(const int *__restrict__ ids, const float *__restrict__ x,
                                                              int ldx, float *__restrict__ out, int L, int D) {
  const int b = blockIdx.x, lane = threadIdx.x;
  int best = INT_MIN, pos = 0;
  for (int l = lane; l < L; l += 64) {
    const int v = ids[(long)b * L + l];
    if (v > best) { best = v; pos = l; }
  }
  for (int o = 32; o > 0; o >>= 1) {
    const int ob = __shfl_xor(best, o), op = __shfl_xor(pos, o);
    if (ob > best || (ob == best && op < pos)) { best = ob; pos = op; }
  }
  const float *src = x + ((long)b * L + pos) * ldx;
  for (int d = lane; d < D; d += 64) out[(long)b * D + d] = src[d];
}

extern "C" int sgic_gather_eot_rows(const int *d_ids, const float *d_x, int ldx, float *d_out, int B, int L, int D,
                                    sgic_stream_t stream) {
  SGIC_REQUIRE(d_ids && d_x && d_out && B > 0 && L > 0 && D > 0 && ldx >= D, "args");
  gather_eot_rows_kernel<<<B, 64, 0, to_stream(stream)>>>(d_ids, d_x, ldx, d_out, L, D);
  return sgic::check_launch("gather_eot_rows_kernel");
}

__global__ void pad_replicate_kernel(const float *__restrict__ in, float *__restrict__ out, int BC, int H, int W, int pl,
                                     int pt, int OH, int OW) {
  const long total = (long)BC * OH * OW;
  GRID_STRIDE(i, total) {
    const int ox = (int)(i % OW);
    long t = i / OW;
    const int oy = (int)(t % OH);
    const long bc = t / OH;
    const int sy = min(max(oy - pt, 0), H - 1), sx = min(max(ox - pl, 0), W - 1);
    out[i] = in[(bc * H + sy) * W + sx];
  }
}

extern "C" int sgic_pad_replicate(const float *d_in, float *d_out, int BC, int H, int W, int pl, int pr, int pt, int pb,
                                  sgic_stream_t stream) {
  SGIC_REQUIRE(d_in && d_out && d_in != d_out && BC > 0 && H > 0 && W > 0 && pl >= 0 && pr >= 0 && pt >= 0 && pb >= 0, "args");
  const int OH = H + pt + pb, OW = W + pl + pr;
  pad_replicate_kernel<<<ew_grid((long)BC * OH * OW), 256, 0, to_stream(stream)>>>(d_in, d_out, BC, H, W, pl, pt, OH, OW);
  return sgic::check_launch("pad_replicate_kernel");
}

__global__ void u8hwc_to_f32chw_pad_kernel(const uint8_t *__restrict__ in, float *__restrict__ out, int B, int H, int W, int pl,
                                           int pt, int OH, int OW) {
  const long total = (long)B * 3 * OH * OW;
  GRID_STRIDE(i, total) {
    const int ox = (int)(i % OW);
    long t = i / OW;
    const int oy = (int)(t % OH);
    t /= OH;
    const int c = (int)(t % 3);
    const long b = t / 3;
    const int sy = min(max(oy - pt, 0), H - 1), sx = min(max(ox - pl, 0), W - 1);
    const float v = (float)in[((b * H + sy) * W + sx) * 3 + c];
    out[i] = __fdiv_rn(v, 255.0f) * 2.0f - 1.0f;
  }
}

extern "C" int sgic_u8hwc_to_f32chw_pad(const uint8_t *d_in, float *d_out, int B, int H, int W, int pl, int pr, int pt, int pb,
                                        sgic_stream_t stream) {
  SGIC_REQUIRE(d_in && d_out && B > 0 && H > 0 && W > 0 && pl >= 0 && pr >= 0 && pt >= 0 && pb >= 0, "args");
  const int OH = H + pt + pb, OW = W + pl + pr;
  u8hwc_to_f32chw_pad_kernel<<<ew_grid((long)B * 3 * OH * OW), 256, 0, to_stream(stream)>>>(d_in, d_out, B, H, W, pl, pt, OH, OW);
  return sgic::check_launch("u8hwc_to_f32chw_pad_kernel");
}

#define RAGGED_CHUNK 32

struct RaggedExtents {
// ... 428 lines not shown
```

### searchable-generative-image-compression_amd/encoder.py

```python
import numpy as np
import torch

from . import ops
from .config import CodecConfig


def _dev(t, device):
    return t.to(device=device, dtype=torch.float32).contiguous()


class RabW:

    def __init__(self, sd, p, device):
        g = lambda k: _dev(sd[f"{p}.{k}"], device)
        self.ln1w, self.ln1b = g("ln_1.weight"), g("ln_1.bias")
        self.inw, self.inb = g("attn.in_proj_weight"), g("attn.in_proj_bias")
        self.ow, self.ob = g("attn.out_proj.weight"), g("attn.out_proj.bias")
        self.ln2w, self.ln2b = g("ln_2.weight"), g("ln_2.bias")
        self.fcw, self.fcb = g("mlp.c_fc.weight"), g("mlp.c_fc.bias")
        self.pjw, self.pjb = g("mlp.c_proj.weight"), g("mlp.c_proj.bias")


def rab_forward(X, w: RabW, L, nseq, heads, bias=None):
    D = X.shape[1]
    h = ops.layernorm(X, w.ln1w, w.ln1b, to_gemm=True)
    qkv = ops.gemm(h, w.inw, w.inb)
    att = ops.attention(qkv[:, 0:D], qkv[:, D:2 * D], qkv[:, 2 * D:3 * D], h, L, nseq, heads, bias=bias, to_gemm=True)
    ops.gemm(att, w.ow, w.ob, residual=X, out=X)
    h = ops.layernorm(X, w.ln2w, w.ln2b, out=h, to_gemm=True)
    f = ops.gemm(h, w.fcw, w.fcb, act=ops.ACT_GELU, to_gemm=True)
    ops.gemm(f, w.pjw, w.pjb, residual=X, out=X)
    return X


def rab_forward_last(X, w: RabW, L, nseq, heads, tok0, Lq, keep=None, bias=None):
    D = X.shape[1]
    keep = Lq if keep is None else keep
    assert 0 < keep <= Lq and tok0 + Lq <= L
    h = ops.layernorm(X, w.ln1w, w.ln1b, to_gemm=True)
    kv = ops.gemm(h, w.inw[D:], w.inb[D:])
    hq = ops.layernorm(X[tok0:], w.ln1w, w.ln1b, M=nseq * Lq, x_seg=(Lq, L), to_gemm=True)
    q = ops.gemm(hq, w.inw[:D], w.inb[:D])
    Xq = ops.copy_row_blocks(X[tok0:], keep, L, nseq)
    if keep == Lq:
        att = ops.attention(q, kv[:, 0:D], kv[:, D:2 * D], hq, L, nseq, heads, bias=bias, to_gemm=True, window=(tok0, Lq))
        ops.gemm(att, w.ow, w.ob, residual=Xq, out=Xq)
    else:
        att = ops.attention(q, kv[:, 0:D], kv[:, D:2 * D], None, L, nseq, heads, bias=bias, window=(tok0, Lq))
        ops.gemm(att, w.ow, w.ob, residual=Xq, out=Xq, M=nseq * keep, a_seg=(keep, Lq))
    h = ops.layernorm(Xq, w.ln2w, w.ln2b, to_gemm=True)
    f = ops.gemm(h, w.fcw, w.fcb, act=ops.ACT_GELU, to_gemm=True)
    ops.gemm(f, w.pjw, w.pjb, residual=Xq, out=Xq)
    return Xq


def rel_indices(win):
    idx = torch.tensor([[x, y] for x in range(win) for y in range(win)])
    return idx[None, :, :] - idx[:, None, :] + win - 1


class SwinW:

    def __init__(self, sd, p, shifted, rel, win, device):
        g = lambda k: _dev(sd[f"{p}.{k}"], device)
        self.shifted = shifted
        self.n1w, self.n1b = g("norm_attn.weight"), g("norm_attn.bias")
        self.qkvw = g("attention_block.to_qkv.weight")
        self.ow, self.ob = g("attention_block.to_out.weight"), g("attention_block.to_out.bias")
        self.n2w, self.n2b = g("norm_mlp.weight"), g("norm_mlp.bias")
        self.w0, self.b0 = g("mlp_block.net.0.weight"), g("mlp_block.net.0.bias")
        self.w2, self.b2 = g("mlp_block.net.2.weight"), g("mlp_block.net.2.bias")
        pos = sd[f"{p}.attention_block.pos_embedding"].float()
        if rel:
            ri = rel_indices(win)
            pos = pos[ri[:, :, 0], ri[:, :, 1]]
        if shifted:
            ul = sd[f"{p}.attention_block.upper_lower_mask"].float()
            lr = sd[f"{p}.attention_block.left_right_mask"].float()
            bias = torch.stack([pos, pos + ul, pos + lr, (pos + ul) + lr])
        else:
            bias = pos[None]
        self.bias = _dev(bias, device)


_ROWMAP_CACHE = {}


def swin_rowmap(B, H, W, win, shifted, device):
    key = (B, H, W, win, shifted, str(device))
    if key not in _ROWMAP_CACHE:
        nh, nw = H // win, W // win
        s = win // 2 if shifted else 0
        b, wy, wx, i, j = np.meshgrid(np.arange(B), np.arange(nh), np.arange(nw), np.arange(win), np.arange(win), indexing="ij")
        y = (wy * win + i + s) % H
        x = (wx * win + j + s) % W
        nH, nW = H // 16, W // 16
        row = (((b * nH + y // 16) * nW + x // 16) << 8) + ((y % 16) << 4) + (x % 16)
        var = np.zeros((B, nh, nw), dtype=np.int32)
        if shifted:
            var[:, nh - 1, :] |= 1
            var[:, :, nw - 1] |= 2
        _ROWMAP_CACHE[key] = (torch.from_numpy(row.reshape(-1).astype(np.int32)).to(device),
                              torch.from_numpy(var.reshape(-1)).to(device))
    return _ROWMAP_CACHE[key]


def swin_forward(Fm, w: SwinW, B, H, W, win=16):
    C = Fm.shape[1]
    rowmap, var = swin_rowmap(B, H, W, win, w.shifted, Fm.device)
    h = ops.layernorm(Fm, w.n1w, w.n1b, to_gemm=True)
    qkv = ops.gemm(h, w.qkvw)
    nseq = B * (H // win) * (W // win)
    att = ops.attention(qkv[:, 0:C], qkv[:, C:2 * C], qkv[:, 2 * C:3 * C], h, win * win, nseq, C // 64, rowmap=rowmap,
                        bias=w.bias, biasvar=var if w.shifted else None, to_gemm=True)
    ops.gemm(att, w.ow, w.ob, residual=Fm, out=Fm)
    h = ops.layernorm(Fm, w.n2w, w.n2b, out=h, to_gemm=True)
    f = ops.gemm(h, w.w0, w.b0, act=ops.ACT_GELU, to_gemm=True)
    ops.gemm(f, w.w2, w.b2, residual=Fm, out=Fm)
    return Fm


def swin_stack_weights(sd, p, n, win, device, first_index=1):
    return [SwinW(sd, f"{p}.{first_index + i}", bool(i % 2), i == 0, win, device) for i in range(n)]


class ConvNextW:
    def __init__(self, sd, p, device):
        g = lambda k: _dev(sd[f"{p}.{k}"], device)
        C = sd[f"{p}.conv.weight"].shape[0]
        self.ls = _dev(sd[f"{p}.layer_scale"].reshape(C), device)
        self.dw = _dev(sd[f"{p}.conv.weight"].reshape(C, 25).t(), device)
        self.db = g("conv.bias")
        self.nw, self.nb = g("norm.weight"), g("norm.bias")
        self.w0, self.b0 = g("mlp.0.weight"), g("mlp.0.bias")
        self.w2, self.b2 = g("mlp.2.weight"), g("mlp.2.bias")


def convnext_forward(Fm, w: ConvNextW, B, H, W):
    t = ops.dwconv(Fm, w.dw, w.db, w.ls, B, H, W, 5, tile16=True)
    t = ops.layernorm(t, w.nw, w.nb, out=t, to_gemm=True)
    f = ops.gemm(t, w.w0, w.b0, act=ops.ACT_GELU, to_gemm=True)
    ops.gemm(f, w.w2, w.b2, residual=Fm, out=Fm)
    return Fm


class CrossW:
    def __init__(self, sd, p, n_attn, device):
        g = lambda k: _dev(sd[f"{p}.{k}"], device)
        self.tpos = _dev(sd[f"{p}.titok_pos_emb"].squeeze(1), device)
        self.fpos = _dev(sd[f"{p}.feat_pos_emb"].squeeze(1), device)
        self.cw, self.cb = g("titok_compress_proj.weight"), g("titok_compress_proj.bias")
        self.attn = [RabW(sd, f"{p}.attn.{j}", device) for j in range(n_attn)]
        self.dw, self.db = g("titok_decompress_proj.0.weight"), g("titok_decompress_proj.0.bias")
        self.dnw, self.dnb = g("titok_decompress_proj.1.weight"), g("titok_decompress_proj.1.bias")
        self.fnw, self.fnb = g("feat_add.0.weight"), g("feat_add.0.bias")
        self.fw, self.fb = g("feat_add.1.weight"), g("feat_add.1.bias")
        self.zw, self.zb = g("zero_add.weight"), g("zero_add.bias")


def cross_forward(Fm, X, w: CrossW, N, Lt, P2):
    Fd = Fm.shape[1]
    LJ = Lt + P2
    J = torch.empty(N * LJ, Fd, device=X.device, dtype=torch.float32)
    tmp = torch.empty_like(X)
    ops.add_rows_bcast(X, Lt, w.tpos, tmp, Lt, N, Lt)
    ops.gemm(tmp, w.cw, w.cb, out=J, M=N * Lt, c_seg=(Lt, LJ))
    ops.add_rows_bcast(Fm, P2, w.fpos, J[Lt:], LJ, N, P2)
    for rw in w.attn:
        rab_forward(J, rw, LJ, N, Fd // 64)
    t = ops.layernorm(J[Lt:], w.fnw, w.fnb, M=N * P2, x_seg=(P2, LJ), to_gemm=True)
    ops.gemm(t, w.fw, w.fb, residual=Fm, out=Fm)
    t = ops.gemm(J, w.dw, w.db, M=N * Lt, a_seg=(Lt, LJ))
    t = ops.layernorm(t, w.dnw, w.dnb, out=t, act=ops.ACT_SILU, to_gemm=True)
    ops.gemm(t, w.zw, w.zb, residual=X, out=X)
    return Fm, X


class HybridEncoderHIP:
    def __init__(self, sd, cfg: CodecConfig, device, p="hybrid_codec.encoder", prune_last=True):
        self.cfg, self.device = cfg, device
        self.prune_last = prune_last
        g = lambda k: _dev(sd[f"{p}.{k}"], device)
        Wd, Fd = cfg.width, cfg.feat_dim
        self.pe_w = _dev(sd[f"{p}.patch_embed.weight"].reshape(Wd, -1), device)
        self.pe_b = g("patch_embed.bias")
        self.cls, self.pos, self.latpos = g("class_embedding"), g("positional_embedding"), g("latent_token_positional_embedding")
        self.lat = _dev(sd["hybrid_codec.latent_tokens"], device)
        self.lnpre_w, self.lnpre_b = g("ln_pre.weight"), g("ln_pre.bias")
        self.layers = [RabW(sd, f"{p}.transformer.{i}", device) for i in range(cfg.layers)]
        self.lnpost_w, self.lnpost_b = g("ln_post.weight"), g("ln_post.bias")
        self.co_w = _dev(sd[f"{p}.conv_out.weight"].reshape(cfg.token_size, Wd), device)
        self.co_b = g("conv_out.bias")
        self.pix_w = _dev(sd[f"{p}.pix_emb_proj.weight"].reshape(Fd, Wd), device)
        self.pix_b = g("pix_emb_proj.bias")
        self.cross, self.fblocks = {}, {}
        for i in cfg.in_pos_enc:
            self.cross[i] = CrossW(sd, f"{p}.inter_blocks.{i}", cfg.n_attn, device)
            self.fblocks[i] = (swin_stack_weights(sd, f"{p}.feat_blocks.{i}.0", 2, cfg.window, device),
                               ConvNextW(sd, f"{p}.feat_blocks.{i}.1", device), ConvNextW(sd, f"{p}.feat_blocks.{i}.2", device))
        self.feat_in = swin_stack_weights(sd, f"{p}.feat_in", 4, cfg.window, device)
        self.feat_out_swin = swin_stack_weights(sd, f"{p}.feat_out.0", 2, cfg.window, device)
        self.fo_cw = _dev(sd[f"{p}.feat_out.1.weight"].permute(0, 2, 3, 1).reshape(Fd, 4 * Fd), device)
        self.fo_cb = g("feat_out.1.bias")
        self.fo_nw, self.fo_nb = g("feat_out.3.weight"), g("feat_out.3.bias")
        self.fo_lw, self.fo_lb = g("feat_out.4.weight"), g("feat_out.4.bias")

    def forward(self, x, taps=None):
        cfg = self.cfg
        B, _, H, W = x.shape
        P, g, T, Wd = cfg.patch_size, cfg.grid, cfg.num_latent_tokens, cfg.width
        Hf, Wf = H // P, W // P
        nH, nW = Hf // g, Wf // g
        N, P2 = B * nH * nW, g * g
        L = 1 + P2 + T
        A = ops.im2col_patch(x, P, 0.5, 0.5, tile16=True)
        emb = ops.gemm(A, self.pe_w, self.pe_b)
        Fm = ops.gemm(emb, self.pix_w, self.pix_b)
        X = ops.assemble_tokens(emb, self.cls, self.pos, self.lat, self.latpos, N, P2, T, Wd)
        for w in self.feat_in:
            swin_forward(Fm, w, B, Hf, Wf, cfg.window)
        ops.layernorm(X, self.lnpre_w, self.lnpre_b, out=X)
        if taps is not None:
            taps["feat_in"] = Fm.clone()
            taps["x_ln_pre"] = X.clone()
        last = cfg.layers - 1
        prune = self.prune_last and taps is None and last not in self.cross and P2 % 32 == 0
        for i in range(cfg.layers - 1 if prune else cfg.layers):
            rab_forward(X, self.layers[i], L, N, cfg.heads)
            if i in self.cross:
                cross_forward(Fm, X, self.cross[i], N, 1 + P2 + T, P2)
                sw, c1, c2 = self.fblocks[i]
                for w in sw:
                    swin_forward(Fm, w, B, Hf, Wf, cfg.window)
                convnext_forward(Fm, c1, B, Hf, Wf)
                convnext_forward(Fm, c2, B, Hf, Wf)
            if taps is not None and i == 0:
                taps["x_layer0"] = X.clone()
        if prune:
            Xq = rab_forward_last(X, self.layers[last], L, N, cfg.heads, P2, T + 1)
            lat = ops.layernorm(Xq[1:], self.lnpost_w, self.lnpost_b, M=N * T, x_seg=(T, T + 1))
        else:
            lat = ops.layernorm(X[1 + P2:], self.lnpost_w, self.lnpost_b, M=N * T, x_seg=(T, L))
        latT = ops.fake2d_transpose(lat, T * Wd, N, T, Wd)
        z = ops.gemm(latT, self.co_w, self.co_b)
        for w in self.feat_out_swin:
            swin_forward(Fm, w, B, Hf, Wf, cfg.window)
        A2 = ops.im2col_2x2(Fm, B, Hf, Wf, tile16=True)
        h = ops.gemm(A2, self.fo_cw, self.fo_cb)
        ops.layernorm(h, self.fo_nw, self.fo_nb, out=h)
        h = ops.gemm(h, self.fo_lw, self.fo_lb)
        return z, h, (nH, nW)
```

### searchable-generative-image-compression_amd/ops.py

```python
import ctypes
import json
import math
import os

import numpy as np
import torch

from ._lib import call, check, launch_opts, lib, require_gpu

ACT_NONE, ACT_GELU, ACT_SILU, ACT_TANH, ACT_LRELU = 0, 1, 2, 3, 4

PROFILE = None
_PROFILER = None


def _profiler():
    global _PROFILER
    if _PROFILER is None:
        h = ctypes.c_void_p(0)
        check(lib.sgic_profiler_create(ctypes.byref(h)), "sgic_profiler_create")
        _PROFILER = h
    return _PROFILER


# ... 84 lines not shown
def save_tile_cache(path=None):
    global _DIRTY
    if not _DIRTY and path is None:
        return None
    finalize_autotune()
    path = path or _user_cache_path()
    picks = {}
    try:
        with open(path) as f:
            picks = json.load(f).get("picks", {})
    except (OSError, ValueError):
        pass
    picks.update({"|".join(str(int(x)) if not isinstance(x, str) else x for x in k): int(v) for k, v in _TILE.items()})
    try:
        os.makedirs(os.path.dirname(path), exist_ok=True)
        tmp = f"{path}.{os.getpid()}.tmp"
        with open(tmp, "w") as f:
            json.dump({"device": "gfx950", "format": "kind|M|...: launch mode (sgic_launch_opts)", "picks": dict(sorted(picks.items()))}, f, indent=0)
        os.replace(tmp, path)
    except OSError:
        return None
    _DIRTY = False
    return path


def _lookup(key):
    m = _TILE.get(key)
    if m is not None:
        return m
    fam = _FAMILY.get((key[0],) + tuple(key[2:]))
    if fam:
        M = key[1]
        near = min(fam, key=lambda x: abs(x - M))
        if M <= 2 * near and near <= 2 * M:
            _TILE[key] = fam[near]
            return fam[near]
    return None


def tile_of(key, dev=None):
    if key and key[0] == "batched":
        return 0
    if key and key[0] in ("conv3x3", "conv3"):
        return _TILE.get(key)
    M, N, K, res, act = key[:5]
    kind = "gemm3" if len(key) > 5 and key[5] == "s3" else "gemm"
    return _TILE.get((kind, M, N, K, int(bool(res)), act))


_load_tile_cache()


def _save_at_exit():
    try:
        if _DIRTY:
            save_tile_cache()
    except Exception:
        pass


import atexit

atexit.register(_save_at_exit)


_TUNE_PROF = None


def _tune_profiler():
    global _TUNE_PROF
    if _TUNE_PROF is None:
        h = ctypes.c_void_p(0)
        check(lib.sgic_profiler_create(ctypes.byref(h)), "sgic_profiler_create")
        _TUNE_PROF = h
    return _TUNE_PROF


def _tune(key, launch, modes=None):
    prof = _tune_profiler()
    modes = TUNE_MODES if modes is None else modes
    reps = 3
    times = {}
    for _ in range(2):
        if M_big(key):
            for mode in modes:
                launch(mode)
                e0, e1 = torch.cuda.Event(enable_timing=True), torch.cuda.Event(enable_timing=True)
                e0.record()
                for _ in range(4):
                    launch(mode)
                e1.record()
                e1.synchronize()
                t = e0.elapsed_time(e1)
                times[mode] = min(t, times.get(mode, t))
            continue
        check(lib.sgic_profiler_begin(prof, len(modes) * reps), "sgic_profiler_begin")
        for mode in modes:
            launch(mode)
            for _ in range(reps):
                launch(mode, prof)
        buf = (ctypes.c_float * (len(modes) * reps))()
        n = ctypes.c_int(0)
        check(lib.sgic_profiler_end(prof, buf, len(modes) * reps, ctypes.byref(n)), "sgic_profiler_end")
        if n.value != len(modes) * reps:
            raise RuntimeError(f"tile tuner: {n.value} timed launches, expected {len(modes) * reps}")
        for i, mode in enumerate(modes):
            t = min(buf[i * reps + r] for r in range(reps))
            times[mode] = min(t, times.get(mode, t))
    order = sorted(times, key=times.get)
    best = order[0]
    _remember(key, best)
    cands = [m for m in order[:CTX_CANDS] if times[m] <= 1.06 * times[best]]
    if CTX_REPS > 0 and len(cands) > 1 and M_big(key):
        _CTX[key] = {"cands": cands, "t": {m: [] for m in cands}, "i": 0}
    return best


CTX_CANDS, CTX_REPS = 3, 2
_CTX = {}


def M_big(key):
    if key[0] in ("conv3x3", "conv3"):
        return True
    return 2.0 * key[1] * key[2] * key[3] >= 5e9


def _ctx_launch(key, launch):
    c = _CTX[key]
    mode = c["cands"][c["i"] % len(c["cands"])]
    c["i"] += 1
    e0, e1 = torch.cuda.Event(enable_timing=True), torch.cuda.Event(enable_timing=True)
    e0.record()
    launch(mode)
    e1.record()
    e1.synchronize()
    c["t"][mode].append(e0.elapsed_time(e1))
    if c["i"] >= len(c["cands"]) * CTX_REPS:
        _remember(key, min(c["cands"], key=lambda m: min(c["t"][m])))
        del _CTX[key]


def finalize_autotune():
    for key in list(_CTX):
        c = _CTX.pop(key)
        done = [m for m in c["cands"] if c["t"][m]]
        if done:
            _remember(key, min(done, key=lambda m: min(c["t"][m])))


def _pick_and_launch(key, launch, big_enough, restore=None, modes=None):
    tile = 0
    if big_enough:
        tile = _lookup(key)
        if tile is None:
            if not AUTOTUNE or PROFILE is not None:
                tile = 0
            elif restore is not None:
                saved = restore.clone()
                tile = _tune(key, launch, modes)
                restore.copy_(saved)
            else:
                tile = _tune(key, launch, modes)
        elif key in _CTX and PROFILE is None:
            _ctx_launch(key, launch)
            return True
    global LAST_TILE
    LAST_TILE = tile
    launch(tile)
    return False


LAST_TILE = 0
PROFILE_TILES = []


PRECISION = os.environ.get("SGIC_GEMM", "split3")
assert PRECISION in ("f32", "split3"), f"SGIC_GEMM={PRECISION!r}: expected f32 or split3"
SPLIT3_MODES = (1, 2, 3, 4, 5, 6, 7, 8, 9, 10, 11, 12, 13, 14, 15, 16, 17, 18, 19, 20, 21, 22, 23, 24, 25, 26, 27, 28, 29, 30, 31)
SPLIT3_RING_MODES = (18, 19, 20, 21, 22, 23, 24, 25)
SPLIT3_SMALL_M = 2048


def _split3_modes(M):
    return SPLIT3_MODES if M <= SPLIT3_SMALL_M else tuple(m for m in SPLIT3_MODES if m not in SPLIT3_RING_MODES)


_W3 = {}
_W3_BYTES = 0
_W3_LIMIT = 24 << 30
_A3_WS = {}


def set_precision(p):
    global PRECISION
    assert p in ("f32", "split3"), p
    PRECISION = p


class Planes:
    __slots__ = ("t", "rows", "cols")

    def __init__(self, rows, cols, device, buf=None):
        n = 3 * rows * cols
        if buf is not None and buf.numel() >= n:
            self.t = buf
        else:
            self.t = torch.empty(n, device=device, dtype=torch.int16)
        self.rows, self.cols = rows, cols

    @property
    def shape(self):
        return (self.rows, self.cols)

    @property
    def device(self):
        return self.t.device

    def rowmajor(self):
        p = self.t[:3 * self.rows * self.cols].view(3, self.cols // 32, self.rows, 32)
        return p.permute(0, 2, 1, 3).reshape(3, self.rows, self.cols)

    def float(self):
        p = self.rowmajor()
        f = lambda q: (q.to(torch.int32) << 16).view(torch.float32)
        return (f(p[0]) + f(p[1])) + f(p[2])


def planes_ok(cols, precision=None):
    return (precision or PRECISION) == "split3" and cols % 32 == 0


def split3(x, ld=None, rows=None, seg=(0, 0), out=None):
    x, ldx = _rows(x)
    rows = x.shape[0] if rows is None else rows
    cols = x.shape[1]
    if out is None:
        out = torch.empty(3, rows, cols, device=x.device, dtype=torch.int16)
    call("sgic_split3_f32", _p(x), ldx if ld is None else ld, rows, cols, seg[0], seg[1], _p(out))
    return out


def split3_planes(x, out=None):
    x, ldx = _rows(x)
    rows, cols = x.shape
    assert cols % 32 == 0
    pl = out if isinstance(out, Planes) and out.shape == (rows, cols) else Planes(rows, cols, x.device)
    call("sgic_split3_pack_f32", _p(x), ldx, rows, cols, _p(pl.t))
    return pl


def weight_planes(w, ldw):
    global _W3_BYTES
    N, K = w.shape
    key = (w.data_ptr(), N, K, ldw, w._version)
    hit = _W3.get(key)
    if hit is None:
        planes = torch.empty(3, N, K, device=w.device, dtype=torch.int16)
        call("sgic_split3_pack_f32", _p(w), ldw, N, K, _p(planes))
        nbytes = planes.numel() * 2
        while _W3 and _W3_BYTES + nbytes > _W3_LIMIT:
            old = next(iter(_W3))
            _W3_BYTES -= _W3.pop(old)[0].numel() * 2
        _W3[key] = hit = (planes, w)
        _W3_BYTES += nbytes
    return hit[0]


def _a3_workspace(dev, n_u16):
    key = (dev, _stream_key())
    ws = _A3_WS.get(key)
    if ws is None or ws.numel() < n_u16:
        ws = torch.empty(max(n_u16, 1 << 24), device=dev, dtype=torch.int16)
        _A3_WS[key] = ws
    return ws


def _stream_key():
    from ._lib import stream
    return stream().value


def gemm(a, w, bias=None, residual=None, act=ACT_NONE, out=None, M=None, a_seg=(0, 0), c_seg=(0, 0), tile=None, w_const=True,
         precision=None, to_gemm=False):
    require_gpu()
    a_planes = a if isinstance(a, Planes) else None
    if a_planes is not None:
        K, lda = a_planes.cols, a_planes.cols
        assert a_seg[0] == 0 and (M is None or M == a_planes.rows)
        M = a_planes.rows
        dev = a_planes.device
    else:
        a, lda = _rows(a)
        K = a.shape[1]
        if M is None:
            M = a.shape[0]
        dev = a.device
    w, ldw = _rows(w)
    N = w.shape[0]
    assert w.shape[1] == K, ((M, K), w.shape)
    use3 = (precision or PRECISION) == "split3" and w_const and K % 32 == 0
    assert a_planes is None or use3, "a Planes operand needs the split path"
    out_planes = None
    if to_gemm and use3 and N % 32 == 0 and c_seg[0] == 0:
        out_planes = out if isinstance(out, Planes) and out.shape == (M, N) else Planes(M, N, dev, buf=out.t if isinstance(out, Planes) else None)
        out, ldc = None, N
    else:
        if isinstance(out, Planes):
            out = None
        if out is None:
            assert c_seg[0] == 0
            out = torch.empty(M, N, device=dev, dtype=torch.float32)
        out, ldc = _rows(out)
        assert out.shape[1] == N
    ldr = 0
    if residual is not None:
        residual, ldr = _rows(residual)
        assert residual.shape[1] == N and residual.shape[0] >= M
    if bias is not None:
        assert bias.shape == (N,) and bias.is_contiguous()
    inplace = residual is not None and out is not None and out.data_ptr() == residual.data_ptr()

    if use3:
        wp = weight_planes(w, ldw)
        ap = a_planes.t if a_planes is not None else _a3_workspace(dev, 3 * M * K)
        a_f32 = None if a_planes is not None else a
        cp = out_planes.t if out_planes is not None else None

        def launch3(mode, prof=None):
            call("sgic_gemm_split3_f32", _p(a_f32), lda, a_seg[0], a_seg[1], _p(ap), _p(wp), _p(bias), _p(residual), ldr, _p(out), ldc,
                 _p(cp), M, N, K, act, c_seg[0], c_seg[1], _opts(tile=mode, prof=prof, w_packed=1, a_packed=1))

        if tile is not None:
            launch3(tile)
        else:
            key = ("gemm3", M, N, K, int(residual is not None), act)
            if _pick_and_launch(key, launch3, M * N >= (1 << 16), restore=out if inplace else None, modes=_split3_modes(M)):
                return out_planes if out_planes is not None else out
        if PROFILE is not None:
            PROFILE.append((2.0 * M * N * K, (M, N, K, residual is not None, act, "s3")))
            PROFILE_TILES.append(tile if tile is not None else LAST_TILE)
        return out_planes if out_planes is not None else out

    def launch(mode, prof=None):
        call("sgic_gemm_f32", _p(a), lda, _p(w), ldw, _p(bias), _p(residual), ldr, _p(out), ldc, M, N, K, act,
             a_seg[0], a_seg[1], c_seg[0], c_seg[1], _opts(tile=mode, prof=prof))

    if tile is not None:
        launch(tile)
    else:
        key = ("gemm", M, N, K, int(residual is not None), act)
        if _pick_and_launch(key, launch, M * N >= (1 << 16), restore=out if inplace else None):
            return out
    if PROFILE is not None:
        PROFILE.append((2.0 * M * N * K, (M, N, K, residual is not None, act)))
        PROFILE_TILES.append(tile if tile is not None else LAST_TILE)
    return out


def layernorm(x, gamma, beta, out=None, eps=1e-5, act=ACT_NONE, M=None, x_seg=(0, 0), y_seg=(0, 0), to_gemm=False):
    x, ldx = _rows(x)
    C = x.shape[1]
    if M is None:
        M = x.shape[0]
    assert gamma.shape == (C,) and beta.shape == (C,)
    if to_gemm and planes_ok(C) and C % 256 == 0 and C <= 2048 and y_seg[0] == 0:
        pl = out if isinstance(out, Planes) and out.shape == (M, C) else Planes(M, C, x.device, buf=out.t if isinstance(out, Planes) else None)
        call("sgic_layernorm_split3_f32", _p(x), ldx, x_seg[0], x_seg[1], _p(gamma), _p(beta), _p(pl.t), M, C, float(eps), act)
        return pl
    if isinstance(out, Planes):
        out = None
    if out is None:
        assert y_seg[0] == 0
        out = torch.empty(M, C, device=x.device, dtype=torch.float32)
    out, ldy = _rows(out)
    call("sgic_layernorm_f32", _p(x), ldx, x_seg[0], x_seg[1], _p(gamma), _p(beta), _p(out), ldy, y_seg[0], y_seg[1],
         M, C, float(eps), act)
    return out


def attention(q, k, v, out, L, nseq, nheads, rowmap=None, bias=None, biasvar=None, scale=0.125, mode=None, to_gemm=False, precision=None,
              window=None):
    q, ldq = _rows(q)
    k, ldk = _rows(k)
    v, ldv = _rows(v)
    D = nheads * 64
    pl = None
    if to_gemm and planes_ok(D):
        rows = q.shape[0]
        pl = out if isinstance(out, Planes) and out.shape == (rows, D) else Planes(rows, D, q.device, buf=out.t if isinstance(out, Planes) else None)
    else:
        if out is None or isinstance(out, Planes):
            out = torch.empty(q.shape[0], D, device=q.device, dtype=torch.float32)
        out, ldo = _rows(out)
    if rowmap is not None:
        assert rowmap.dtype == torch.int32 and rowmap.numel() == nseq * L and rowmap.is_contiguous()
    q_tok0, Lq = window if window is not None else (0, 0)
    if window is not None:
        assert Lq > 0 and q.shape[0] >= nseq * Lq and (pl is not None or out.shape[0] >= nseq * Lq), (window, q.shape)
    win = "_window" if window is not None else ""
    wargs = (int(q_tok0), int(Lq)) if window is not None else ()
    if bias is not None:
        assert bias.dim() == 3 and bias.shape[1] == L and bias.shape[2] == L and bias.is_contiguous()
    if biasvar is not None:
        assert biasvar.dtype == torch.int32 and biasvar.numel() == nseq

    s3 = 8 if (precision or PRECISION) == "split3" else 0

    def launch(m):
        if pl is not None:
            call(f"sgic_attention{win}_split3_f32", _p(q), ldq, _p(k), ldk, _p(v), ldv, _p(pl.t), ctypes.c_long(pl.rows), L, nseq, nheads,
                 _p(rowmap), _p(bias), _p(biasvar), float(scale), *wargs, launch_opts(0, m | s3, None))
        else:
            call(f"sgic_attention{win}_f32", _p(q), ldq, _p(k), ldk, _p(v), ldv, _p(out), ldo, L, nseq, nheads, _p(rowmap), _p(bias),
                 _p(biasvar), float(scale), *wargs, launch_opts(0, m | s3, None))

    if mode is None:
        mode = 0
        if nseq * nheads * L >= 4096:
            key = ("attn3" if s3 else "attn", nseq, L, nheads, int(bias is not None)) + wargs
            mode = _lookup(key)
            if mode is None:
                mode = 0
                if AUTOTUNE and PROFILE is None:
                    best_t = None
                    for cand in ATTN_MODES:
                        launch(cand)
                        e0, e1 = torch.cuda.Event(enable_timing=True), torch.cuda.Event(enable_timing=True)
                        e0.record()
                        for _ in range(3):
                            launch(cand)
                        e1.record()
                        e1.synchronize()
                        t = e0.elapsed_time(e1)
                        if best_t is None or t < best_t:
                            mode, best_t = cand, t
                    _remember(key, mode)
    launch(mode)
    return pl if pl is not None else out


def copy_row_blocks(x, rows, stride_rows, nblocks, out=None):
    x, ldx = _rows(x)
    C = x.shape[1]
    assert ldx == C and stride_rows >= rows and x.shape[0] >= (nblocks - 1) * stride_rows + rows, (x.shape, rows, stride_rows, nblocks)
    if out is None:
        out = torch.empty(nblocks * rows, C, device=x.device, dtype=torch.float32)
    assert out.is_contiguous() and out.shape == (nblocks * rows, C)
    call("sgic_copy_blocks_f32", _p(x), _cl(stride_rows * C), _p(out), _cl(rows * C), _cl(rows * C), nblocks)
    return out


def im2col_patch(x, P, mul=1.0, add=0.0, tile16=False, out=None):
    assert x.dim() == 4 and x.is_contiguous() and x.dtype == torch.float32
    B, C, H, W = x.shape
    if out is None:
        out = torch.empty(B * (H // P) * (W // P), C * P * P, device=x.device, dtype=torch.float32)
    call("sgic_im2col_patch", _p(x), B, C, H, W, P, float(mul), float(add), int(tile16), _p(out))
    return out


def assemble_tokens(emb, cls, pos, lat, latpos, N, P, T, D, out=None):
    if out is None:
        out = torch.empty(N * (1 + P + T), D, device=emb.device, dtype=torch.float32)
    call("sgic_assemble_tokens", _p(emb), _p(cls), _p(pos), _p(lat), _p(latpos), N, P, T, D, _p(out))
    return out


def add_rows_bcast(inp, iseg, vec, out, oseg, Nn, Lr):
    inp, ldi = _rows(inp)
    out, ldo = _rows(out)
    D = inp.shape[1]
    assert out.shape[1] == D
    if vec is not None:
        assert vec.is_contiguous() and vec.numel() == Lr * D
    call("sgic_add_rows_bcast", _p(inp), ldi, iseg, _p(vec), _p(out), ldo, oseg, Nn, Lr, D)
    return out


def dwconv(x, w_kkc, bias, prescale, B, H, W, k, tile16=False, out=None):
    x, ldx = _rows(x)
    C = x.shape[1]
    assert ldx == C and w_kkc.shape == (k * k, C) and w_kkc.is_contiguous()
    if out is None:
        out = torch.empty_like(x)
    call("sgic_dwconv_nhwc", _p(x), _p(w_kkc), _p(bias), _p(prescale), _p(out), B, H, W, C, k, int(tile16))
    return out


def im2col_2x2(x, B, H, W, tile16=False, out=None):
    x, ldx = _rows(x)
    C = x.shape[1]
    assert ldx == C
    if out is None:
        out = torch.empty(B * (H // 2) * (W // 2), 4 * C, device=x.device, dtype=torch.float32)
    call("sgic_im2col_2x2", _p(x), B, H, W, C, int(tile16), _p(out))
    return out


def gated_lrelu(x, out=None):
    x, ldx = _rows(x)
    M, C2x2 = x.shape
    assert ldx == C2x2
    if out is None:
        out = torch.empty(M, C2x2 // 2, device=x.device, dtype=torch.float32)
    call("sgic_gated_lrelu", _p(x), _p(out), M, C2x2 // 2)
    return out


def colop(x, v, mode, out=None):
    x, ldx = _rows(x)
    v, ldv = _rows(v)
    M, C = x.shape
    if out is None:
        out = torch.empty(M, C, device=x.device, dtype=torch.float32)
    out, ldy = _rows(out)
    call("sgic_colop", _p(x), ldx, _p(v), ldv, v.shape[0], _p(out), ldy, M, C, mode)
    return out


def fake2d_transpose(x_base, seq_stride, N, T, D):
    out = torch.empty(N * T, D, device=x_base.device, dtype=torch.float32)
    call("sgic_fake2d_transpose", _p(x_base), _cl(seq_stride), _p(out), N, T, D)
    return out


def vq_argmin(z, codebook, l2norm=True):
    z, ldz = _rows(z)
    M, dim = z.shape
    assert codebook.is_contiguous() and codebook.shape[1] == dim
    idx = torch.empty(M, dtype=torch.int32, device=z.device)
    call("sgic_vq_argmin", _p(z), ldz, _p(codebook), codebook.shape[0], dim, M, int(l2norm), _p(idx))
    return idx


def l2norm_u8(x):
    x, ldx = _rows(x)
    M, D = x.shape
    unit = torch.empty(M, D, device=x.device, dtype=torch.float32)
    q = torch.empty(M, D, device=x.device, dtype=torch.uint8)
    call("sgic_l2norm_u8", _p(x), ldx, M, D, _p(unit), _p(q))
    return unit, q


def quant_step(y, scales, means, ld_sm, yhat, ld_yhat, B, H, W, C, k, thr, sym, idx):
    call("sgic_quant_step", _p(y), _p(scales), _p(means), ld_sm, _p(yhat), ld_yhat, B, H, W, C, k,
         float(-1.0 if thr is None else thr), _p(sym), _p(idx))


def scale_indexes(scales_flat, idx_out, thr):
    call("sgic_scale_to_index", _p(scales_flat), _cl(scales_flat.numel()), float(-1.0 if thr is None else thr), _p(idx_out))


def index_step(scales, ld_sm, B, H, W, C, k, thr, idx):
    call("sgic_index_step", _p(scales), ld_sm, B, H, W, C, k, float(-1.0 if thr is None else thr), _p(idx))


def index_margins(scales, ld_sm, B, H, W, C, k, thr, margin, alt):
    call("sgic_index_margins", _p(scales), ld_sm, B, H, W, C, k, float(-1.0 if thr is None else thr), _p(margin), _p(alt))


def dequant_step(sym, means, ld_sm, yhat, ld_yhat, B, H, W, C, k):
    call("sgic_dequant_step", _p(sym), _p(means), ld_sm, _p(yhat), ld_yhat, B, H, W, C, k)


def rans_encode_batch(table, sym, idx, B, n, cap=None):
    if cap is None:
        cap = 2 * n + 64
    dev = sym.device
    out = torch.empty(B, cap, dtype=torch.uint8, device=dev)
    meta = torch.empty(3, B, dtype=torch.int32, device=dev)
    call("sgic_rans_encode_batch", table, _p(sym), _p(idx), B, n, _p(out), cap, _p(meta[0]), _p(meta[1]), _p(meta[2]))
    return out, meta


def pack12_batch(idx_i32, B, n):
    nb = lib.sgic_pack12_size(n)
    out = torch.empty(B, nb, dtype=torch.uint8, device=idx_i32.device)
    call("sgic_pack12_batch", _p(idx_i32), B, n, _p(out))
    return out


def gemm_batched(a, lda, sa, w, ldw, sw, out, ldc, sc, M, N, K, batch, bias=None, residual=None, ldr=0, sr=0, act=ACT_NONE):
    call("sgic_gemm_batched_f32", _p(a), lda, _cl(sa), _p(w), ldw, _cl(sw), _p(bias), _p(residual), ldr, _cl(sr), _p(out), ldc,
         _cl(sc), M, N, K, act, batch, _opts())
    if PROFILE is not None:
        PROFILE.append((2.0 * M * N * K * batch, ("batched", batch, M, N, K, residual is not None, act)))
        PROFILE_TILES.append(0)
    return out


class HaloPlanes:
    __slots__ = ("t", "B", "H", "W", "C")

    def __init__(self, t, B, H, W, C):
        self.t, self.B, self.H, self.W, self.C = t, B, H, W, C


_HALO3 = {}


def halo_planes_buffer(dev, B, H, W, C):
    key = (str(dev), B, H, W, C)
    if key not in _HALO3:
        _HALO3[key] = HaloPlanes(torch.zeros(3 * B * (H + 2) * (W + 2) * C, device=dev, dtype=torch.int16), B, H, W, C)
    return _HALO3[key]


def conv_planes_ok(Cin, Cout, residual=False, precision=None):
    return (precision or PRECISION) == "split3" and Cin % 32 == 0 and not (Cout == 3 and Cin == 128 and not residual)


def conv3x3(x_halo, w, bias, B, H, W, Cin, Cout, residual=None, act=ACT_NONE, out=None, tile=None, precision=None):
    hp = x_halo if isinstance(x_halo, HaloPlanes) else None
    if hp is not None:
        assert (hp.B, hp.H, hp.W, hp.C) == (B, H, W, Cin) and conv_planes_ok(Cin, Cout, residual is not None, precision)
        dev = hp.t.device
    else:
        assert x_halo.is_contiguous() and x_halo.numel() == B * (H + 2) * (W + 2) * Cin
        dev = x_halo.device
    assert w.shape == (Cout, 9 * Cin) and w.is_contiguous()
    if out is None:
        out = torch.empty(B * H * W, Cout, device=dev, dtype=torch.float32)
    out, ldc = _rows(out)
    ldr = 0
    if residual is not None:
        residual, ldr = _rows(residual)

    if conv_planes_ok(Cin, Cout, residual is not None, precision):
        rows = B * (H + 2) * (W + 2)
        wp = weight_planes(w, 9 * Cin)
        if hp is not None:
            ws = hp.t
        else:
            ws = _a3_workspace(dev, 3 * rows * Cin)
            call("sgic_split3_pack_f32", _p(x_halo), Cin, rows, Cin, _p(ws))

        def launch3(mode, prof=None):
            call("sgic_conv3x3_split3_f32", _p(ws), _p(wp), _p(bias), _p(residual), ldr, _p(out), ldc, B, H, W, Cin, Cout, act,
                 _opts(tile=mode, prof=prof, w_packed=1, a_packed=1))

        if tile is not None:
            launch3(tile)
        else:
            key = ("conv3", B * H * W, H, W, Cin, Cout, int(residual is not None), act)
            if _pick_and_launch(key, launch3, B * H * W * Cout >= (1 << 20), modes=(1, 2, 3, 5, 10, 11, 14, 15, 16, 17, 30)):
                return out
        if PROFILE is not None:
            PROFILE.append((2.0 * B * H * W * Cout * 9 * Cin, (B * H * W, Cout, 9 * Cin, residual is not None, act, "s3", "conv")))
            PROFILE_TILES.append(tile if tile is not None else LAST_TILE)
        return out

    def launch(mode, prof=None):
        call("sgic_conv3x3_f32", _p(x_halo), _p(w), _p(bias), _p(residual), ldr, _p(out), ldc, B, H, W, Cin, Cout, act,
             _opts(tile=mode, prof=prof))

    if tile is not None:
        launch(tile)
    else:
        key = ("conv3x3", B * H * W, H, W, Cin, Cout, int(residual is not None), act)
        if _pick_and_launch(key, launch, B * H * W * Cout >= (1 << 20)):
            return out
    if PROFILE is not None:
        PROFILE.append((2.0 * B * H * W * Cout * 9 * Cin, (B * H * W, Cout, 9 * Cin, residual is not None, act, "f32", "conv")))
        PROFILE_TILES.append(tile if tile is not None else LAST_TILE)
    return out


_GN_WS = {}


def groupnorm(x, gamma, beta, B, H, W, swish=True, halo=False, groups=32, eps=1e-6, out=None, to_conv=None):
    x, ldx = _rows(x)
    C = x.shape[1]
    assert ldx == C
    dev = x.device
    key = (str(dev), B, C)
    if key not in _GN_WS:
        _GN_WS[key] = (torch.empty(B * 64 * C * 2, dtype=torch.float64, device=dev),
                       torch.empty(B * groups * 2, dtype=torch.float32, device=dev))
    ws, stats = _GN_WS[key]
    if halo and to_conv is not None and conv_planes_ok(C, to_conv[0], to_conv[1]):
        hp = halo_planes_buffer(dev, B, H, W, C)
        call("sgic_groupnorm_nhwc_split3", _p(x), _p(gamma), _p(beta), B, H, W, C, groups, float(eps), int(swish), _p(ws), _p(stats),
             _p(hp.t))
        return hp
    if out is None:
        out = halo_buffer(dev, B, H, W, C) if halo else torch.empty(B * H * W, C, device=dev)
    call("sgic_groupnorm_nhwc", _p(x), _p(gamma), _p(beta), B, H, W, C, groups, float(eps), int(swish), int(halo), _p(ws),
         _p(stats), _p(out))
    return out


_HALO = {}


def halo_buffer(dev, B, H, W, C):
    key = (str(dev), B, H, W, C)
    if key not in _HALO:
        _HALO[key] = torch.zeros(B, H + 2, W + 2, C, device=dev, dtype=torch.float32)
    return _HALO[key]


def halo_copy(x, B, H, W, C, upsample=False, tile16=False, out=None, to_conv=None):
    s = 2 if upsample else 1
    if to_conv is not None and conv_planes_ok(C, to_conv[0], to_conv[1]):
        hp = halo_planes_buffer(x.device, B, H * s, W * s, C)
        call("sgic_halo_copy_split3", _p(x), B, H, W, C, int(upsample), int(tile16), _p(hp.t))
        return hp
    if out is None:
        out = halo_buffer(x.device, B, H * s, W * s, C)
    call("sgic_halo_copy", _p(x), B, H, W, C, int(upsample), int(tile16), _p(out))
    return out


def softmax_rows(x, L, scale=1.0, out=None):
    assert x.is_contiguous()
    M = x.numel() // L
    if out is None:
        out = torch.empty_like(x)
    call("sgic_softmax_rows", _p(x), _p(out), _cl(M), L, float(scale))
    return out


def pixel_shuffle2_tm16(x, B, H, W, C):
    out = torch.empty(B * 4 * H * W, C, device=x.device, dtype=torch.float32)
    call("sgic_pixel_shuffle2_tm16", _p(x), B, H, W, C, _p(out))
    return out


def assemble_dec_tokens(emb, cls, mask, pos, latpos, N, P, T, D):
    out = torch.empty(N * (1 + P + T), D, device=emb.device, dtype=torch.float32)
    call("sgic_assemble_dec_tokens", _p(emb), _p(cls), _p(mask), _p(pos), _p(latpos), N, P, T, D, _p(out))
    return out


def codebook_gather_norm(idx, codebook, ld=None):
    M, dim = idx.numel(), codebook.shape[1]
    ld = ld or dim
    out = torch.empty(M, ld, device=idx.device, dtype=torch.float32)
    call("sgic_codebook_gather_norm", _p(idx), _p(codebook), M, dim, ld, _p(out))
    return out


def nhwc3_to_nchw_clamp(x, ld, B, H, W):
    out = torch.empty(B, 3, H, W, device=x.device, dtype=torch.float32)
    call("sgic_nhwc3_to_nchw_clamp", _p(x), ld, B, H, W, _p(out))
    return out


def rans_decode_init(streams, cap, off, ln, B):
    state = torch.zeros(B, 4, dtype=torch.int32, device=streams.device)
    call("sgic_rans_decode_init_batch", _p(streams), cap, _p(off), _p(ln), B, _p(state))
    return state


def rans_decode_step(table, streams, cap, off, ln, B, state, idx, n, idx_stride, out, out_stride):
    call("sgic_rans_decode_batch", table, _p(streams), cap, _p(off), _p(ln), B, _p(state), _p(idx), n, idx_stride, _p(out),
         out_stride)


def unpack12_batch(streams_u8, B, n):
    out = torch.empty(B, n, dtype=torch.int32, device=streams_u8.device)
    call("sgic_unpack12_batch", _p(streams_u8), B, n, _p(out))
    return out


def pad_replicate(x, pl, pr, pt, pb):
    assert x.dim() == 4 and x.is_contiguous() and x.dtype == torch.float32
    B, C, H, W = x.shape
    if pl == pr == pt == pb == 0:
        return x
    out = torch.empty(B, C, H + pt + pb, W + pl + pr, device=x.device, dtype=torch.float32)
    call("sgic_pad_replicate", _p(x), _p(out), B * C, H, W, int(pl), int(pr), int(pt), int(pb))
    return out


def u8hwc_to_f32chw_pad(x_u8, pl=0, pr=0, pt=0, pb=0):
    assert x_u8.dim() == 4 and x_u8.shape[3] == 3 and x_u8.dtype == torch.uint8 and x_u8.is_contiguous() and x_u8.is_cuda
    B, H, W, _ = x_u8.shape
    out = torch.empty(B, 3, H + pt + pb, W + pl + pr, device=x_u8.device, dtype=torch.float32)
    call("sgic_u8hwc_to_f32chw_pad", _p(x_u8), _p(out), B, H, W, int(pl), int(pr), int(pt), int(pb))
    return out


def u8canvas_to_f32chw_pad(x_u8, hw, OH, OW):
    assert x_u8.dim() == 4 and x_u8.shape[3] == 3 and x_u8.dtype == torch.uint8 and x_u8.is_contiguous() and x_u8.is_cuda
    B, Hc, Wc, _ = x_u8.shape
    hw = np.ascontiguousarray(hw, dtype=np.int32).reshape(B, 2)
    out = torch.empty(B, 3, int(OH), int(OW), device=x_u8.device, dtype=torch.float32)
    call("sgic_u8canvas_to_f32chw_pad", _p(x_u8), hw, _p(out), B, Hc, Wc, int(OH), int(OW))
    return out


def clip_preprocess_u8canvas(x_u8, geo, S, mean, std):
    assert x_u8.dim() == 4 and x_u8.shape[3] == 3 and x_u8.dtype == torch.uint8 and x_u8.is_contiguous() and x_u8.is_cuda
    B, Hc, Wc, _ = x_u8.shape
    geo = np.ascontiguousarray(geo, dtype=np.int32).reshape(B, 6)
    mean, std = (np.ascontiguousarray(v, dtype=np.float32).reshape(3) for v in (mean, std))
    nbytes = ctypes.c_size_t(0)
    call("sgic_clip_preprocess_u8canvas_workspace", B, geo, int(S), ctypes.byref(nbytes))
    work = torch.empty(nbytes.value, dtype=torch.uint8, device=x_u8.device)
    out = torch.empty(B, 3, int(S), int(S), dtype=torch.float32, device=x_u8.device)
    call("sgic_clip_preprocess_u8canvas", _p(x_u8), Hc, Wc, B, geo, int(S), mean, std, _p(work), ctypes.c_size_t(nbytes.value), _p(out))
    return out


def clip_resize_coeffs(in_size, out_size, device):
    ksize = int(np.ceil(2.0 * max(in_size / out_size, 1.0))) * 2 + 1
    bounds = torch.empty(out_size, 2, dtype=torch.int32, device=device)
    kk = torch.empty(out_size, ksize, dtype=torch.int32, device=device)
    call("sgic_clip_resize_coeffs", int(in_size), int(out_size), ksize, _p(bounds), _p(kk))
    return bounds, kk, ksize


def topk_rows(scores, k):
    nq, n = scores.shape
    assert scores.is_contiguous()
    os_ = torch.empty(nq, k, device=scores.device, dtype=torch.float32)
    oi = torch.empty(nq, k, device=scores.device, dtype=torch.int32)
    call("sgic_topk_rows", _p(scores), nq, n, k, _p(os_), _p(oi))
    return os_, oi


# ... 152 lines not shown
```

Before: 520.9 images/s.

## Emit split3 GEMM operand planes directly from producer kernels and GEMM epilogues

```diff
diff --git a/include/sgic.h b/include/sgic.h
--- a/include/sgic.h
+++ b/include/sgic.h
@@ -105,6 +105,13 @@
                int mode, sgic_stream_t stream);
 int sgic_fake2d_transpose(const float *d_in, long in_seq_stride, float *d_out, int N, int T, int D,
                           sgic_stream_t stream);
+int sgic_im2col_patch_split3(const float *d_x, int B, int C, int H, int W, int P, float mul, float add, int tile16,
+                             uint16_t *d_planes, sgic_stream_t stream);
+int sgic_add_rows_bcast_split3(const float *d_in, int ldi, int iseg, const float *d_vec, uint16_t *d_planes, int Nn, int Lr,
+                               int D, sgic_stream_t stream);
+int sgic_im2col_2x2_split3(const float *d_x, int B, int H, int W, int C, int tile16, uint16_t *d_planes, sgic_stream_t stream);
+int sgic_fake2d_transpose_split3(const float *d_in, long in_seq_stride, uint16_t *d_planes, int N, int T, int D,
+                                 sgic_stream_t stream);
 int sgic_vq_argmin(const float *d_z, int ldz, const float *d_codebook, int ncodes, int dim, int M, int l2norm,
                    int32_t *d_idx, sgic_stream_t stream);
 int sgic_clip_preprocess(const float *d_x, long img_stride, long ch_stride, int ldx, int B, int H, int W, int OH,
diff --git a/searchable-generative-image-compression_amd/clip.py b/searchable-generative-image-compression_amd/clip.py
--- a/searchable-generative-image-compression_amd/clip.py
+++ b/searchable-generative-image-compression_amd/clip.py
@@ -134,7 +134,7 @@
         B = pre.shape[0]
         g = cfg.image_size // cfg.patch
         L = g * g + 1
-        A = ops.im2col_patch(pre, cfg.patch, 1.0, 0.0, tile16=False)
+        A = ops.im2col_patch(pre, cfg.patch, 1.0, 0.0, tile16=False, to_gemm=True)
         emb = ops.gemm(A, self.conv_w)
         X = ops.assemble_tokens(emb, self.cls, self.pos, None, None, B, g * g, 0, cfg.width)
         ops.layernorm(X, self.lnpre_w, self.lnpre_b, out=X)
@@ -142,11 +142,11 @@
             for w in self.blocks[:-1]:
                 rab_forward(X, w, L, B, cfg.heads)
             pooled = rab_forward_last(X, self.blocks[-1], L, B, cfg.heads, 0, 32, keep=1)
-            ops.layernorm(pooled, self.lnpost_w, self.lnpost_b, out=pooled)
+            pooled = ops.layernorm(pooled, self.lnpost_w, self.lnpost_b, to_gemm=True)
         else:
             for w in self.blocks:
                 rab_forward(X, w, L, B, cfg.heads)
-            pooled = ops.layernorm(X, self.lnpost_w, self.lnpost_b, M=B, x_seg=(1, L))
+            pooled = ops.layernorm(X, self.lnpost_w, self.lnpost_b, M=B, x_seg=(1, L), to_gemm=True)
         z = ops.gemm(pooled, self.projT)
         return ops.l2norm_u8(z)
 
diff --git a/searchable-generative-image-compression_amd/csrc/gemm_split.hip b/searchable-generative-image-compression_amd/csrc/gemm_split.hip
--- a/searchable-generative-image-compression_amd/csrc/gemm_split.hip
+++ b/searchable-generative-image-compression_amd/csrc/gemm_split.hip
@@ -70,64 +70,80 @@
     const int nc = colok ? n : 0;
     f32x4 bv = {0.f, 0.f, 0.f, 0.f};
     if (g.bias && colok) bv = *reinterpret_cast<const f32x4 *>(g.bias + n);
-    s3_for<PASSES>([&](auto pass_c) __attribute__((always_inline)) {
-      constexpr int pass = decltype(pass_c)::value;
-#pragma unroll
-      for (int i = 0; i < BMP; i++)
-#pragma unroll
-        for (int j = 0; j < BN; j++) *reinterpret_cast<f32x4 *>(ep + (i * 16 + l16) * LDW + j * 16 + 4 * lq) = acc[pass * BMP + i][j];
-      asm volatile("s_waitcnt lgkmcnt(0)" ::: "memory");
-      const int wmp = wm + pass * RM;
-      auto run = [&](auto act_c, auto res_c, auto pl_c) __attribute__((always_inline)) {
-        constexpr int ACT = decltype(act_c)::value;
-        constexpr bool HASR = decltype(res_c)::value != 0, PLANES = decltype(pl_c)::value != 0;
-        constexpr int EB = NIT < 8 ? NIT : 8;
-#pragma unroll
-        for (int b = 0; b < NIT; b += EB) {
-          f32x4 cv[EB], rv[EB];
+    auto run = [&](auto act_c, auto res_c, auto pl_c) __attribute__((always_inline)) {
+      constexpr int ACT = decltype(act_c)::value;
+      constexpr bool HASR = decltype(res_c)::value != 0;
+      constexpr int OUT = decltype(pl_c)::value;
+      constexpr int EB = BM * BN > 16 ? 4 : (NIT < 8 ? NIT : 8);
+      constexpr int NB = (NIT + EB - 1) / EB, NCH = PASSES * NB, DEPTH = NCH < 2 ? NCH : 2;
+      f32x4 rv[HASR ? DEPTH : 1][EB];
+      auto load_r = [&](auto ch_c) __attribute__((always_inline)) {
+        constexpr int ch = decltype(ch_c)::value, wmp = (ch / NB) * RM, b = (ch % NB) * EB;
+#pragma unroll
+        for (int q = 0; q < EB; ++q) {
+          const int rr = EXACT ? (b + q) * RPI + r0 : min((b + q) * RPI + r0, RM - 1);
+          rv[ch % DEPTH][q] = *reinterpret_cast<const f32x4 *>(g.R + (size_t)(min(em0 + wm + wmp + rr, g.M - 1) + g.m_base) * g.ldr + nc);
+        }
+      };
+      if constexpr (HASR) s3_for<DEPTH>(load_r);
+      s3_for<PASSES>([&](auto pass_c) __attribute__((always_inline)) {
+        constexpr int pass = decltype(pass_c)::value;
+#pragma unroll
+        for (int i = 0; i < BMP; i++)
+#pragma unroll
+          for (int j = 0; j < BN; j++) *reinterpret_cast<f32x4 *>(ep + (i * 16 + l16) * LDW + j * 16 + 4 * lq) = acc[pass * BMP + i][j];
+        asm volatile("s_waitcnt lgkmcnt(0)" ::: "memory");
+        const int wmp = wm + pass * RM;
+        s3_for<NB>([&](auto b_c) __attribute__((always_inline)) {
+          constexpr int ch = pass * NB + decltype(b_c)::value, b = decltype(b_c)::value * EB;
+          f32x4 cv[EB];
 #pragma unroll
           for (int q = 0; q < EB; ++q) {
             const int rr = EXACT ? (b + q) * RPI + r0 : min((b + q) * RPI + r0, RM - 1);
             cv[q] = *reinterpret_cast<const f32x4 *>(ep + rr * LDW + c4);
-            if constexpr (HASR) rv[q] = *reinterpret_cast<const f32x4 *>(g.R + (size_t)(min(em0 + wmp + rr, g.M - 1) + g.m_base) * g.ldr + nc);
           }
+#pragma unroll
+          for (int q = 0; q < EB; ++q) {
+#pragma unroll
+            for (int t = 0; t < 4; t++) cv[q][t] = apply_act_c<ACT>(cv[q][t] + bv[t]);
+            if constexpr (HASR) cv[q] += rv[ch % DEPTH][q];
+          }
+          if constexpr (HASR && ch + DEPTH < NCH) load_r(IntC<ch + DEPTH>{});
 #pragma unroll
           for (int q = 0; q < EB; ++q) {
             if (!EXACT && (b + q >= NIT || (b + q) * RPI + r0 >= RM)) continue;
             const int m = em0 + wmp + (b + q) * RPI + r0;
-            f32x4 v = cv[q];
-#pragma unroll
-            for (int t = 0; t < 4; t++) v[t] = apply_act_c<ACT>(v[t] + bv[t]);
-            if constexpr (HASR) v += rv[q];
             if (colok && m < g.M) {
-              if constexpr (PLANES) {
-                s3_store4(g.Cp, g.c_plane, s3_pack_off(m + g.m_base, n, g.c_rows), v);
-              } else {
+              if constexpr (OUT != 0) s3_store4(g.Cp, g.c_plane, s3_pack_off(m + g.m_base, n, g.c_rows), cv[q]);
+              if constexpr (OUT != 1) {
                 const int mm = m + g.m_base;
                 const size_t crow = g.c_seg ? (size_t)(mm / g.c_seg) * g.c_seg_stride + (mm % g.c_seg) : (size_t)mm;
-                *reinterpret_cast<f32x4 *>(g.C + crow * g.ldc + n) = v;
+                *reinterpret_cast<f32x4 *>(g.C + crow * g.ldc + n) = cv[q];
               }
             }
           }
-        }
-      };
-      auto run_act = [&](auto act_c) __attribute__((always_inline)) {
-        if (g.Cp) {
-          if (g.R) run(act_c, IntC<1>{}, IntC<1>{});
-          else run(act_c, IntC<0>{}, IntC<1>{});
-        } else {
-          if (g.R) run(act_c, IntC<1>{}, IntC<0>{});
-          else run(act_c, IntC<0>{}, IntC<0>{});
-        }
-      };
-      switch (g.act) {
-        case ACT_GELU: run_act(IntC<ACT_GELU>{}); break;
-        case ACT_SILU: run_act(IntC<ACT_SILU>{}); break;
-        case ACT_TANH: run_act(IntC<ACT_TANH>{}); break;
-        case ACT_LRELU: run_act(IntC<ACT_LRELU>{}); break;
-        default: run_act(IntC<ACT_NONE>{}); break;
-      }
-    });
+        });
+      });
+    };
+    auto run_act = [&](auto act_c) __attribute__((always_inline)) {
+      if (g.Cp && g.C) {
+        if (g.R) run(act_c, IntC<1>{}, IntC<2>{});
+        else run(act_c, IntC<0>{}, IntC<2>{});
+      } else if (g.Cp) {
+        if (g.R) run(act_c, IntC<1>{}, IntC<1>{});
+        else run(act_c, IntC<0>{}, IntC<1>{});
+      } else {
+        if (g.R) run(act_c, IntC<1>{}, IntC<0>{});
+        else run(act_c, IntC<0>{}, IntC<0>{});
+      }
+    };
+    switch (g.act) {
+      case ACT_GELU: run_act(IntC<ACT_GELU>{}); break;
+      case ACT_SILU: run_act(IntC<ACT_SILU>{}); break;
+      case ACT_TANH: run_act(IntC<ACT_TANH>{}); break;
+      case ACT_LRELU: run_act(IntC<ACT_LRELU>{}); break;
+      default: run_act(IntC<ACT_NONE>{}); break;
+    }
     return;
   }
   auto run = [&](auto act_c, auto res_c) __attribute__((always_inline)) {
@@ -996,7 +1012,7 @@
   SGIC_REQUIRE(d_Aplanes && d_Wplanes && (d_C || d_Cplanes) && M > 0 && N > 0 && K > 0, "null/empty");
   SGIC_REQUIRE((K & 31) == 0, "K must be a multiple of 32");
   SGIC_REQUIRE(((uintptr_t)d_Aplanes & 15) == 0 && ((uintptr_t)d_Wplanes & 15) == 0, "planes must be 16-byte aligned");
-  SGIC_REQUIRE((d_Cplanes || ldc >= N) && (!d_R || ldr >= N), "leading dimensions");
+  SGIC_REQUIRE((!d_C || ldc >= N) && (!d_R || ldr >= N), "leading dimensions");
   SGIC_REQUIRE(act >= 0 && act <= ACT_LRELU, "activation");
   SGIC_REQUIRE(c_seg >= 0 && (c_seg == 0 || c_seg_stride >= c_seg), "row segment map");
   int a_packed = opts ? opts->a_packed : 0;
@@ -1010,7 +1026,7 @@
   }
   SGIC_REQUIRE(!d_Cplanes || (N & 31) == 0, "planes output needs N % 32 == 0");
   const int vec = (N % 4 == 0) && (!d_bias || ((uintptr_t)d_bias & 15) == 0) && (!d_R || ((ldr % 4 == 0) && ((uintptr_t)d_R & 15) == 0)) &&
-                  (d_Cplanes ? ((uintptr_t)d_Cplanes & 7) == 0 : ((ldc % 4 == 0) && ((uintptr_t)d_C & 15) == 0));
+                  (!d_Cplanes || ((uintptr_t)d_Cplanes & 7) == 0) && (!d_C || ((ldc % 4 == 0) && ((uintptr_t)d_C & 15) == 0));
   SGIC_REQUIRE(!d_Cplanes || (vec && c_seg == 0), "planes output needs float4-addressable operands and no row map");
   S3Args g{d_Aplanes, d_Wplanes, d_bias, d_R, d_C, M, N, K, ldr, ldc, act, c_seg, c_seg_stride, (long)M * K, (long)N * K, d_Cplanes, (long)M * N, vec, 0, 0, 0, 0,
            opts ? opts->w_packed : 0, a_packed, M, M};
diff --git a/searchable-generative-image-compression_amd/csrc/misc.hip b/searchable-generative-image-compression_amd/csrc/misc.hip
--- a/searchable-generative-image-compression_amd/csrc/misc.hip
+++ b/searchable-generative-image-compression_amd/csrc/misc.hip
@@ -1,12 +1,46 @@
 #include "common.h"
+#include "split3.h"
 #include <limits.h>
 
 typedef float f32x4 __attribute__((ext_vector_type(4)));
+typedef unsigned u32x4 __attribute__((ext_vector_type(4)));
 
 __device__ __forceinline__ long fmap_row(int b, int y, int x, int H, int W, int tile16) {
   if (!tile16) return ((long)b * H + y) * W + x;
   const int nH = H >> 4, nW = W >> 4;
   return ((((long)b * nH + (y >> 4)) * nW + (x >> 4)) << 8) + ((y & 15) << 4) + (x & 15);
+}
+
+__device__ __forceinline__ void fmap_row_inv(long row, int H, int W, int tile16, int &b, int &y, int &x) {
+  if (!tile16) {
+    x = (int)(row % W);
+    row /= W;
+    y = (int)(row % H);
+    b = (int)(row / H);
+    return;
+  }
+  const int nH = H >> 4, nW = W >> 4, in = (int)(row & 255);
+  row >>= 8;
+  x = (int)(row % nW) * 16 + (in & 15);
+  row /= nW;
+  y = (int)(row % nH) * 16 + (in >> 4);
+  b = (int)(row / nH);
+}
+
+__device__ __forceinline__ void planes_index(long i, long rows, long &row, int &col) {
+  row = (i >> 2) % rows;
+  col = (int)((i >> 2) / rows) * 32 + (int)(i & 3) * 8;
+}
+__device__ __forceinline__ void planes_store8(unsigned short *planes, long rows, int cols, long row, int col, const f32x4 &v0, const f32x4 &v1) {
+  unsigned p1[4], p2[4], p3[4];
+  s3_split_pair(v0[0], v0[1], p1[0], p2[0], p3[0]);
+  s3_split_pair(v0[2], v0[3], p1[1], p2[1], p3[1]);
+  s3_split_pair(v1[0], v1[1], p1[2], p2[2], p3[2]);
+  s3_split_pair(v1[2], v1[3], p1[3], p2[3], p3[3]);
+  const size_t plane = (size_t)rows * cols, dst = s3_pack_off((size_t)row, col, (size_t)rows);
+  *reinterpret_cast<u32x4 *>(planes + dst) = u32x4{p1[0], p1[1], p1[2], p1[3]};
+  *reinterpret_cast<u32x4 *>(planes + plane + dst) = u32x4{p2[0], p2[1], p2[2], p2[3]};
+  *reinterpret_cast<u32x4 *>(planes + 2 * plane + dst) = u32x4{p3[0], p3[1], p3[2], p3[3]};
 }
 
 #define GRID_STRIDE(i, n) for (long i = (long)blockIdx.x * blockDim.x + threadIdx.x; i < (n); i += (long)gridDim.x * blockDim.x)
@@ -47,6 +81,37 @@
   const long total = (long)B * (H / P) * (W / P) * C * P * (P / 4);
   im2col_patch_kernel<<<ew_grid(total), 256, 0, to_stream(stream)>>>(d_x, B, C, H, W, P, mul, add, tile16, d_out);
   return sgic::check_launch("im2col_patch_kernel");
+}
+
+__global__ void im2col_patch_split3_kernel(const float *__restrict__ x, int B, int C, int H, int W, int P, float mul, float add,
+                                           int tile16, unsigned short *__restrict__ planes) {
+  const int gh = H / P, gw = W / P, K = C * P * P;
+  const long rows = (long)B * gh * gw, total = rows * (K >> 3);
+  GRID_STRIDE(i, total) {
+    long row;
+    int col, b, gy, gx;
+    planes_index(i, rows, row, col);
+    fmap_row_inv(row, gh, gw, tile16, b, gy, gx);
+    const int kx = col % P, ky = (col / P) % P, c = col / (P * P);
+    const float *src = x + (((long)b * C + c) * H + gy * P + ky) * W + gx * P + kx;
+    f32x4 v0 = *reinterpret_cast<const f32x4 *>(src), v1 = *reinterpret_cast<const f32x4 *>(src + 4);
+#pragma unroll
+    for (int e = 0; e < 4; e++) {
+      v0[e] = v0[e] * mul + add;
+      v1[e] = v1[e] * mul + add;
+    }
+    planes_store8(planes, rows, K, row, col, v0, v1);
+  }
+}
+
+extern "C" int sgic_im2col_patch_split3(const float *d_x, int B, int C, int H, int W, int P, float mul, float add, int tile16,
+                                        uint16_t *d_planes, sgic_stream_t stream) {
+  SGIC_REQUIRE(d_x && d_planes && B > 0 && C > 0 && P >= 8 && (P & 7) == 0 && H % P == 0 && W % P == 0, "args");
+  SGIC_REQUIRE(!tile16 || ((H / P) % 16 == 0 && (W / P) % 16 == 0), "tile-major order needs a patch grid multiple of 16");
+  SGIC_REQUIRE((W & 3) == 0 && ((uintptr_t)d_x & 15) == 0 && ((uintptr_t)d_planes & 15) == 0 && (C * P * P) % 32 == 0, "alignment");
+  const long total = (long)B * (H / P) * (W / P) * C * P * (P / 8);
+  im2col_patch_split3_kernel<<<ew_grid(total), 256, 0, to_stream(stream)>>>(d_x, B, C, H, W, P, mul, add, tile16, d_planes);
+  return sgic::check_launch("im2col_patch_split3_kernel");
 }
 
 __global__ void assemble_tokens_kernel(const float *__restrict__ emb, const float *__restrict__ cls,
@@ -107,6 +172,34 @@
   const long total = (long)Nn * Lr * (D / 4);
   add_rows_bcast_kernel<<<ew_grid(total), 256, 0, to_stream(stream)>>>(d_in, ldi, iseg, d_vec, d_out, ldo, oseg, Nn, Lr, D);
   return sgic::check_launch("add_rows_bcast_kernel");
+}
+
+__global__ void add_rows_bcast_split3_kernel(const float *__restrict__ in, int ldi, int iseg, const float *__restrict__ vec,
+                                             unsigned short *__restrict__ planes, int Nn, int Lr, int D) {
+  const long rows = (long)Nn * Lr, total = rows * (D >> 3);
+  GRID_STRIDE(i, total) {
+    long row;
+    int col;
+    planes_index(i, rows, row, col);
+    const int l = (int)(row % Lr);
+    const long n = row / Lr;
+    const float *src = in + (n * iseg + l) * ldi + col;
+    f32x4 v0 = *reinterpret_cast<const f32x4 *>(src), v1 = *reinterpret_cast<const f32x4 *>(src + 4);
+    if (vec) {
+      v0 += *reinterpret_cast<const f32x4 *>(vec + (long)l * D + col);
+      v1 += *reinterpret_cast<const f32x4 *>(vec + (long)l * D + col + 4);
+    }
+    planes_store8(planes, rows, D, row, col, v0, v1);
+  }
+}
+
+extern "C" int sgic_add_rows_bcast_split3(const float *d_in, int ldi, int iseg, const float *d_vec, uint16_t *d_planes, int Nn,
+                                          int Lr, int D, sgic_stream_t stream) {
+  SGIC_REQUIRE(d_in && d_planes && Nn > 0 && Lr > 0 && D > 0 && (D & 31) == 0 && (ldi & 3) == 0 && ldi >= D && iseg >= Lr, "args");
+  SGIC_REQUIRE(((uintptr_t)d_in & 15) == 0 && (!d_vec || ((uintptr_t)d_vec & 15) == 0) && ((uintptr_t)d_planes & 15) == 0, "alignment");
+  const long total = (long)Nn * Lr * (D / 8);
+  add_rows_bcast_split3_kernel<<<ew_grid(total), 256, 0, to_stream(stream)>>>(d_in, ldi, iseg, d_vec, d_planes, Nn, Lr, D);
+  return sgic::check_launch("add_rows_bcast_split3_kernel");
 }
 
 __global__ void dwconv_kernel(const float *__restrict__ x, const float *__restrict__ w, const float *__restrict__ bias,
@@ -226,6 +319,31 @@
   return sgic::check_launch("im2col_2x2_kernel");
 }
 
+__global__ void im2col_2x2_split3_kernel(const float *__restrict__ x, int B, int H, int W, int C, int tile16,
+                                         unsigned short *__restrict__ planes) {
+  const int OH = H >> 1, OW = W >> 1;
+  const long rows = (long)B * OH * OW, total = rows * (4 * C >> 3);
+  GRID_STRIDE(i, total) {
+    long row;
+    int col, b, oy, ox;
+    planes_index(i, rows, row, col);
+    fmap_row_inv(row, OH, OW, 0, b, oy, ox);
+    const int kk = col / C, c = col - kk * C;
+    const float *src = x + fmap_row(b, oy * 2 + (kk >> 1), ox * 2 + (kk & 1), H, W, tile16) * C + c;
+    planes_store8(planes, rows, 4 * C, row, col, *reinterpret_cast<const f32x4 *>(src), *reinterpret_cast<const f32x4 *>(src + 4));
+  }
+}
+
+extern "C" int sgic_im2col_2x2_split3(const float *d_x, int B, int H, int W, int C, int tile16, uint16_t *d_planes,
+                                      sgic_stream_t stream) {
+  SGIC_REQUIRE(d_x && d_planes && B > 0 && H > 0 && W > 0 && (H & 1) == 0 && (W & 1) == 0 && C > 0 && (C & 7) == 0, "args");
+  SGIC_REQUIRE(!tile16 || (H % 16 == 0 && W % 16 == 0), "tile-major layout needs H,W multiples of 16");
+  SGIC_REQUIRE(((uintptr_t)d_x & 15) == 0 && ((uintptr_t)d_planes & 15) == 0, "alignment");
+  const long total = (long)B * (H / 2) * (W / 2) * (C / 2);
+  im2col_2x2_split3_kernel<<<ew_grid(total), 256, 0, to_stream(stream)>>>(d_x, B, H, W, C, tile16, d_planes);
+  return sgic::check_launch("im2col_2x2_split3_kernel");
+}
+
 __global__ void gated_lrelu_kernel(const float *__restrict__ x, float *__restrict__ out, long M, int C2) {
   const int C4 = C2 >> 2;
   const long total = M * C4;
@@ -288,6 +406,33 @@
   SGIC_REQUIRE(d_in && d_out && N > 0 && T > 0 && D > 0, "args");
   fake2d_transpose_kernel<<<ew_grid((long)N * T * D), 256, 0, to_stream(stream)>>>(d_in, in_seq_stride, d_out, N, T, D);
   return sgic::check_launch("fake2d_transpose_kernel");
+}
+
+__global__ void fake2d_transpose_split3_kernel(const float *__restrict__ in, long in_seq_stride, unsigned short *__restrict__ planes,
+                                               int N, int T, int D) {
+  const long rows = (long)N * T, total = rows * (D >> 3);
+  GRID_STRIDE(i, total) {
+    long row;
+    int col;
+    planes_index(i, rows, row, col);
+    const int t = (int)(row % T);
+    const float *src = in + (row / T) * in_seq_stride + (long)col * T + t;
+    f32x4 v0, v1;
+#pragma unroll
+    for (int e = 0; e < 4; e++) {
+      v0[e] = src[(long)e * T];
+      v1[e] = src[(long)(e + 4) * T];
+    }
+    planes_store8(planes, rows, D, row, col, v0, v1);
+  }
+}
+
+extern "C" int sgic_fake2d_transpose_split3(const float *d_in, long in_seq_stride, uint16_t *d_planes, int N, int T, int D,
+                                            sgic_stream_t stream) {
+  SGIC_REQUIRE(d_in && d_planes && N > 0 && T > 0 && D > 0 && (D & 31) == 0 && in_seq_stride >= (long)T * D, "args");
+  SGIC_REQUIRE(((uintptr_t)d_planes & 15) == 0, "alignment");
+  fake2d_transpose_split3_kernel<<<ew_grid((long)N * T * (D / 8)), 256, 0, to_stream(stream)>>>(d_in, in_seq_stride, d_planes, N, T, D);
+  return sgic::check_launch("fake2d_transpose_split3_kernel");
 }
 
 extern "C" int sgic_copy_blocks_f32(const float *d_src, long src_stride, float *d_dst, long dst_stride, long block_elems,
diff --git a/searchable-generative-image-compression_amd/encoder.py b/searchable-generative-image-compression_amd/encoder.py
--- a/searchable-generative-image-compression_amd/encoder.py
+++ b/searchable-generative-image-compression_amd/encoder.py
@@ -162,8 +162,7 @@
     Fd = Fm.shape[1]
     LJ = Lt + P2
     J = torch.empty(N * LJ, Fd, device=X.device, dtype=torch.float32)
-    tmp = torch.empty_like(X)
-    ops.add_rows_bcast(X, Lt, w.tpos, tmp, Lt, N, Lt)
+    tmp = ops.add_rows_bcast(X, Lt, w.tpos, None, Lt, N, Lt, to_gemm=True)
     ops.gemm(tmp, w.cw, w.cb, out=J, M=N * Lt, c_seg=(Lt, LJ))
     ops.add_rows_bcast(Fm, P2, w.fpos, J[Lt:], LJ, N, P2)
     for rw in w.attn:
@@ -213,9 +212,9 @@
         nH, nW = Hf // g, Wf // g
         N, P2 = B * nH * nW, g * g
         L = 1 + P2 + T
-        A = ops.im2col_patch(x, P, 0.5, 0.5, tile16=True)
-        emb = ops.gemm(A, self.pe_w, self.pe_b)
-        Fm = ops.gemm(emb, self.pix_w, self.pix_b)
+        A = ops.im2col_patch(x, P, 0.5, 0.5, tile16=True, to_gemm=True)
+        emb, emb_a = ops.gemm(A, self.pe_w, self.pe_b, to_gemm="both")
+        Fm = ops.gemm(emb_a, self.pix_w, self.pix_b)
         X = ops.assemble_tokens(emb, self.cls, self.pos, self.lat, self.latpos, N, P2, T, Wd)
         for w in self.feat_in:
             swin_forward(Fm, w, B, Hf, Wf, cfg.window)
@@ -241,12 +240,12 @@
             lat = ops.layernorm(Xq[1:], self.lnpost_w, self.lnpost_b, M=N * T, x_seg=(T, T + 1))
         else:
             lat = ops.layernorm(X[1 + P2:], self.lnpost_w, self.lnpost_b, M=N * T, x_seg=(T, L))
-        latT = ops.fake2d_transpose(lat, T * Wd, N, T, Wd)
+        latT = ops.fake2d_transpose(lat, T * Wd, N, T, Wd, to_gemm=True)
         z = ops.gemm(latT, self.co_w, self.co_b)
         for w in self.feat_out_swin:
             swin_forward(Fm, w, B, Hf, Wf, cfg.window)
-        A2 = ops.im2col_2x2(Fm, B, Hf, Wf, tile16=True)
+        A2 = ops.im2col_2x2(Fm, B, Hf, Wf, tile16=True, to_gemm=True)
         h = ops.gemm(A2, self.fo_cw, self.fo_cb)
-        ops.layernorm(h, self.fo_nw, self.fo_nb, out=h)
+        h = ops.layernorm(h, self.fo_nw, self.fo_nb, to_gemm=True)
         h = ops.gemm(h, self.fo_lw, self.fo_lb)
         return z, h, (nH, nW)
diff --git a/searchable-generative-image-compression_amd/ops.py b/searchable-generative-image-compression_amd/ops.py
--- a/searchable-generative-image-compression_amd/ops.py
+++ b/searchable-generative-image-compression_amd/ops.py
@@ -410,8 +410,11 @@
     use3 = (precision or PRECISION) == "split3" and w_const and K % 32 == 0
     assert a_planes is None or use3, "a Planes operand needs the split path"
     out_planes = None
+    both = to_gemm == "both"
+    assert both or isinstance(to_gemm, bool), to_gemm
     if to_gemm and use3 and N % 32 == 0 and c_seg[0] == 0:
         out_planes = out if isinstance(out, Planes) and out.shape == (M, N) else Planes(M, N, dev, buf=out.t if isinstance(out, Planes) else None)
+    if out_planes is not None and not both:
         out, ldc = None, N
     else:
         if isinstance(out, Planes):
@@ -421,6 +424,7 @@
             out = torch.empty(M, N, device=dev, dtype=torch.float32)
         out, ldc = _rows(out)
         assert out.shape[1] == N
+    result = (out, out_planes if out_planes is not None else out) if both else (out_planes if out_planes is not None else out)
     ldr = 0
     if residual is not None:
         residual, ldr = _rows(residual)
@@ -444,11 +448,11 @@
         else:
             key = ("gemm3", M, N, K, int(residual is not None), act)
             if _pick_and_launch(key, launch3, M * N >= (1 << 16), restore=out if inplace else None, modes=_split3_modes(M)):
-                return out_planes if out_planes is not None else out
+                return result
         if PROFILE is not None:
             PROFILE.append((2.0 * M * N * K, (M, N, K, residual is not None, act, "s3")))
             PROFILE_TILES.append(tile if tile is not None else LAST_TILE)
-        return out_planes if out_planes is not None else out
+        return result
 
     def launch(mode, prof=None):
         call("sgic_gemm_f32", _p(a), lda, _p(w), ldw, _p(bias), _p(residual), ldr, _p(out), ldc, M, N, K, act,
@@ -459,11 +463,11 @@
     else:
         key = ("gemm", M, N, K, int(residual is not None), act)
         if _pick_and_launch(key, launch, M * N >= (1 << 16), restore=out if inplace else None):
-            return out
+            return result
     if PROFILE is not None:
         PROFILE.append((2.0 * M * N * K, (M, N, K, residual is not None, act)))
         PROFILE_TILES.append(tile if tile is not None else LAST_TILE)
-    return out
+    return result
 
 
 def layernorm(x, gamma, beta, out=None, eps=1e-5, act=ACT_NONE, M=None, x_seg=(0, 0), y_seg=(0, 0), to_gemm=False):
@@ -559,9 +563,13 @@
     return out
 
 
-def im2col_patch(x, P, mul=1.0, add=0.0, tile16=False, out=None):
+def im2col_patch(x, P, mul=1.0, add=0.0, tile16=False, out=None, to_gemm=False):
     assert x.dim() == 4 and x.is_contiguous() and x.dtype == torch.float32
     B, C, H, W = x.shape
+    if to_gemm and planes_ok(C * P * P) and P % 8 == 0:
+        pl = Planes(B * (H // P) * (W // P), C * P * P, x.device)
+        call("sgic_im2col_patch_split3", _p(x), B, C, H, W, P, float(mul), float(add), int(tile16), _p(pl.t))
+        return pl
     if out is None:
         out = torch.empty(B * (H // P) * (W // P), C * P * P, device=x.device, dtype=torch.float32)
     call("sgic_im2col_patch", _p(x), B, C, H, W, P, float(mul), float(add), int(tile16), _p(out))
@@ -575,10 +583,19 @@
     return out
 
 
-def add_rows_bcast(inp, iseg, vec, out, oseg, Nn, Lr):
+def add_rows_bcast(inp, iseg, vec, out, oseg, Nn, Lr, to_gemm=False):
     inp, ldi = _rows(inp)
+    D = inp.shape[1]
+    if to_gemm and planes_ok(D) and oseg == Lr:
+        if vec is not None:
+            assert vec.is_contiguous() and vec.numel() == Lr * D
+        pl = Planes(Nn * Lr, D, inp.device)
+        call("sgic_add_rows_bcast_split3", _p(inp), ldi, iseg, _p(vec), _p(pl.t), Nn, Lr, D)
+        return pl
+    if out is None:
+        assert oseg == Lr
+        out = torch.empty(Nn * Lr, D, device=inp.device, dtype=torch.float32)
     out, ldo = _rows(out)
-    D = inp.shape[1]
     assert out.shape[1] == D
     if vec is not None:
         assert vec.is_contiguous() and vec.numel() == Lr * D
@@ -596,10 +613,14 @@
     return out
 
 
-def im2col_2x2(x, B, H, W, tile16=False, out=None):
+def im2col_2x2(x, B, H, W, tile16=False, out=None, to_gemm=False):
     x, ldx = _rows(x)
     C = x.shape[1]
     assert ldx == C
+    if to_gemm and planes_ok(4 * C) and C % 8 == 0:
+        pl = Planes(B * (H // 2) * (W // 2), 4 * C, x.device)
+        call("sgic_im2col_2x2_split3", _p(x), B, H, W, C, int(tile16), _p(pl.t))
+        return pl
     if out is None:
         out = torch.empty(B * (H // 2) * (W // 2), 4 * C, device=x.device, dtype=torch.float32)
     call("sgic_im2col_2x2", _p(x), B, H, W, C, int(tile16), _p(out))
@@ -627,7 +648,11 @@
     return out
 
 
-def fake2d_transpose(x_base, seq_stride, N, T, D):
+def fake2d_transpose(x_base, seq_stride, N, T, D, to_gemm=False):
+    if to_gemm and planes_ok(D):
+        pl = Planes(N * T, D, x_base.device)
+        call("sgic_fake2d_transpose_split3", _p(x_base), _cl(seq_stride), _p(pl.t), N, T, D)
+        return pl
     out = torch.empty(N * T, D, device=x_base.device, dtype=torch.float32)
     call("sgic_fake2d_transpose", _p(x_base), _cl(seq_stride), _p(out), N, T, D)
     return out
```

Measured after the change: 526.0 images/s (median of 6 runs). Within noise of the previous version (+1.0%).
